# Arsham-001/tsu-emulator

Hardware: AMD Instinct MI355X
Metric: spin-updates/sec on L×L 2D Ising Gibbs sweep; achieved HBM GB/s vs peak (higher is better)
Workload: dtype int8

## Files before the change

tsu-emulator_amd/csrc/ising2d_tiled.hip:

```cpp
#include "ising2d.h"

#include <type_traits>
#include <vector>

typedef short v2s __attribute__((ext_vector_type(2)));
typedef unsigned short v2us __attribute__((ext_vector_type(2)));

struct TiledParams {
    const int8_t* src;
    int8_t* dst;
    long long pitch;
    int rows, nchunks;
    int cols;
    int q_shift;
    int tile_h;
    int flex_ty;
    int r_begin, r_end;
    long long row0, total_rows;
    int wrap_rows, ghost;
    int k;
    int tiles_x;
    int ty_first, ty_stride;
    uint32_t k0, k1, sweep0, tag_hi, tag_lo;
    uint32_t tblH0, tblH1, tblL0, tblL1;
    uint32_t t3H0, t3H1, t3L0, t3L1;
    int open;
    uint64_t thr[25];
};

static __device__ __forceinline__ uint32_t perm(uint32_t s0, uint32_t s1, uint32_t sel) {
    return __builtin_amdgcn_perm(s0, s1, sel);
}
static __device__ __forceinline__ uint32_t subsat16(uint32_t a, uint32_t b) {
    return __builtin_bit_cast(uint32_t, __builtin_elementwise_sub_sat(__builtin_bit_cast(v2s, a), __builtin_bit_cast(v2s, b)));
}
static __device__ __forceinline__ uint32_t minu16(uint32_t a, uint32_t b) {
    return __builtin_bit_cast(uint32_t, __builtin_elementwise_min(__builtin_bit_cast(v2us, a), __builtin_bit_cast(v2us, b)));
}

static __device__ __noinline__ u32x4 resolve_ties(u32x4 d, u32x4 w, uint32_t cnt_lo, uint32_t cnt_hi, const uint64_t* s_thr,
                                                  uint32_t cq, uint32_t Rg, uint32_t hs, uint32_t tag_lo, uint32_t k0,
                                                  uint32_t k1, uint32_t edge = 0) {
    const u32x4 l = tsu_philox(cq, Rg, hs, tag_lo, k0, k1);
#define TSU_FIX(DW, WW, LW, CNT, B0, M0)                                                                        \
    _Pragma("unroll") for (int hlf = 0; hlf < 2; ++hlf) {                                                       \
        const uint32_t sh = 16u * hlf;                                                                          \
        if (((DW >> sh) & 0xFFFFu) == 0) {                                                                      \
            const uint32_t c = (CNT >> (8 * (B0 + hlf))) & 0xFFu;                                               \
            const uint32_t m = M0 + hlf;                                                                        \
            const uint32_t deg = 4u - (edge & 1u) - ((m == 0 && (edge & 2u)) ? 1u : 0u) - ((m == (edge >> 4) && (edge & 4u)) ? 1u : 0u); \
            const uint64_t u = ((uint64_t)(((WW >> sh) & 0xFFFFu) ^ 0x8000u) << 16) | ((LW >> sh) & 0xFFFFu);   \
            const uint32_t f = (u < s_thr[deg * 5 + c]) ? 0x8000u : 0x0001u;       \
            DW = (DW & ~(0xFFFFu << sh)) | (f << sh);                                                           \
        }                                                                                                       \
    }
    TSU_FIX(d.x, w.x, l.x, cnt_lo, 0, 0)
    TSU_FIX(d.y, w.y, l.y, cnt_lo, 2, 2)
    TSU_FIX(d.z, w.z, l.z, cnt_hi, 0, 4)
    TSU_FIX(d.w, w.w, l.w, cnt_hi, 2, 6)
#undef TSU_FIX
    return d;
}

struct PhiloxKeys {
    uint32_t a[10], b[10];
};

static __device__ __forceinline__ PhiloxKeys make_keys(uint32_t k0, uint32_t k1) {
    PhiloxKeys K;
#pragma unroll
    for (int r = 0; r < 10; ++r) {
        uint32_t x = k0 + (uint32_t)r * TSU_PHILOX_W0, y = k1 + (uint32_t)r * TSU_PHILOX_W1;
        asm volatile("v_mov_b32 %0, %1" : "=v"(x) : "s"(x));
        asm volatile("v_mov_b32 %0, %1" : "=v"(y) : "s"(y));
        K.a[r] = x;
        K.b[r] = y;
    }
    return K;
}

static __device__ __forceinline__ u32x4 philox_vk(uint32_t c0, uint32_t c1, uint32_t c2, uint32_t c3, const PhiloxKeys& K) {
#pragma unroll
    for (int r = 0; r < 10; ++r) {
        uint64_t p0 = (uint64_t)TSU_PHILOX_M0 * c0;
        uint64_t p1 = (uint64_t)TSU_PHILOX_M1 * c2;
        uint32_t n0 = tsu_xor3((uint32_t)(p1 >> 32), c1, K.a[r]);
        uint32_t n2 = tsu_xor3((uint32_t)(p0 >> 32), c3, K.b[r]);
        c1 = (uint32_t)p1;
        c3 = (uint32_t)p0;
        c0 = n0;
        c2 = n2;
    }
    return u32x4{c0, c1, c2, c3};
}

struct Rows2Ctx {
    const void* Ps;
    void* Pd;
    const uint64_t* s_thr;
    int tr_lo, npairs;
    int rgf;
    int total_rows;
    int rg_tile0, wrap_tr;
    uint32_t hs, tag_hi, tag_lo, k0, k1;
    uint32_t tblH0, tblH1, tblL0, tblL1;
    uint32_t t3H0, t3H1, t3L0, t3L1;
    int last_row;
    bool lft, rgt;
    uint32_t r_par, r_slot;
    uint32_t rm_lo, rm_hi;
    uint64_t vm_e, vm_o;
    int sh_next, sh_prev;
};

static __device__ __forceinline__ u32x4 compare_octet(const u32x4& w, uint32_t cnt_lo, uint32_t cnt_hi, uint32_t tH0,
                                                      uint32_t tH1, uint32_t tL0, uint32_t tL1) {
    const uint32_t Hl = perm(tH1, tH0, cnt_lo), Ll = perm(tL1, tL0, cnt_lo);
    const uint32_t Hh = perm(tH1, tH0, cnt_hi), Lh = perm(tL1, tL0, cnt_hi);
    u32x4 d;
    d.x = subsat16(w.x, perm(Hl, Ll, 0x05010400u));
    d.y = subsat16(w.y, perm(Hl, Ll, 0x07030602u));
    d.z = subsat16(w.z, perm(Hh, Lh, 0x05010400u));
    d.w = subsat16(w.w, perm(Hh, Lh, 0x07030602u));
    return d;
}

static __device__ __forceinline__ u32x4 compare_octet_open(const u32x4& w, uint32_t cnt_lo, uint32_t cnt_hi, const Rows2Ctx& c,
                                                           bool row_edge, bool l0, bool r7) {
    uint32_t Hl = perm(c.tblH1, c.tblH0, cnt_lo), Ll = perm(c.tblL1, c.tblL0, cnt_lo);
    uint32_t Hh = perm(c.tblH1, c.tblH0, cnt_hi), Lh = perm(c.tblL1, c.tblL0, cnt_hi);
    if (row_edge | l0 | r7) {
        const uint32_t rl = r7 ? c.rm_lo : 0u, rh = r7 ? c.rm_hi : 0u;
        const uint32_t il = cnt_lo + ((row_edge && l0) ? 0x00000004u : 0u) + (row_edge ? (rl & 0x04040404u) : 0u);
        const uint32_t ih = cnt_hi + (row_edge ? (rh & 0x04040404u) : 0u);
        const uint32_t ml = row_edge ? 0xFFFFFFFFu : ((l0 ? 0x000000FFu : 0u) | rl), mh = row_edge ? 0xFFFFFFFFu : rh;
        Hl = (Hl & ~ml) | (perm(c.t3H1, c.t3H0, il) & ml);
        Ll = (Ll & ~ml) | (perm(c.t3L1, c.t3L0, il) & ml);
        Hh = (Hh & ~mh) | (perm(c.t3H1, c.t3H0, ih) & mh);
        Lh = (Lh & ~mh) | (perm(c.t3L1, c.t3L0, ih) & mh);
    }
    u32x4 d;
    d.x = subsat16(w.x, perm(Hl, Ll, 0x05010400u));
    d.y = subsat16(w.y, perm(Hl, Ll, 0x07030602u));
    d.z = subsat16(w.z, perm(Hh, Lh, 0x05010400u));
    d.w = subsat16(w.w, perm(Hh, Lh, 0x07030602u));
    return d;
}

static __device__ __forceinline__ bool has_zero_field(const u32x4& d) {
    const uint32_t mn = minu16(minu16(d.x, d.y), minu16(d.z, d.w));
    return ((mn & 0xFFFFu) == 0) | ((mn >> 16) == 0);
}

static __device__ __forceinline__ uint64_t pack_flags(const u32x4& d) {
    const uint32_t nlo = perm(d.y, d.x, 0x0B0A0908u) & 0x01010101u;
    const uint32_t nhi = perm(d.w, d.z, 0x0B0A0908u) & 0x01010101u;
    return (uint64_t)nlo | ((uint64_t)nhi << 32);
}

template <int NO>
static __device__ __forceinline__ void edge_rows(const Rows2Ctx& c, int to_wrap, int tr, int& rga, int& rgb) {
    constexpr int SPAN = 2 * ((NO - 1 + 63) / NO) + 1;
    const int s_off = to_wrap > 0 ? c.rg_tile0 : c.rg_tile0 - c.total_rows;
    rga = tr + s_off;
    rgb = rga + 1;
    if (__builtin_expect((uint32_t)(to_wrap - 1) < (uint32_t)SPAN, 0)) {
        rga = tr + c.rg_tile0;
        asm volatile("" : "+v"(rga));
        rgb = rga + 1;
        if (rga >= c.total_rows) rga -= c.total_rows;
        if (rgb >= c.total_rows) rgb -= c.total_rows;
    }
}

template <int NO, int P0, bool EDGE, bool OPEN, bool SEAM = false>
static __device__ __forceinline__ void sweep_pairs(const Rows2Ctx& c, const PhiloxKeys& K, int tr_first, int tr_end, int step_rows, int oct,
                                                   uint32_t cq) {
    const char* const ps0 = reinterpret_cast<const char*>(c.Ps);
    const int d_off = (int)(reinterpret_cast<const char*>(c.Pd) - ps0);
    const int off_end = tr_end * NO * 8;
    const int off_step = step_rows * NO * 8;
    int off = (tr_first * NO + oct) * 8;
    int rg = EDGE ? tr_first : c.rgf + (tr_first - c.tr_lo);
    int to_wrap = EDGE ? c.wrap_tr - __builtin_amdgcn_readfirstlane(rg) : 0;
#pragma unroll 1
    for (; off < off_end; off += off_step, rg += step_rows, to_wrap -= step_rows) {
        asm volatile("" : "+v"(off), "+v"(rg));
        const char* ps = ps0 + off;
        const uint64_t R0 = *reinterpret_cast<const uint64_t*>(ps - NO * 8), R1 = *reinterpret_cast<const uint64_t*>(ps);
        const uint64_t R2 = *reinterpret_cast<const uint64_t*>(ps + NO * 8), R3 = *reinterpret_cast<const uint64_t*>(ps + 2 * NO * 8);
        const uint32_t A0 = SEAM ? 0u : *reinterpret_cast<const uint32_t*>(ps + (P0 ? 8 : -4));
        const uint32_t A1 = SEAM ? 0u : *reinterpret_cast<const uint32_t*>(ps + NO * 8 + (P0 ? -4 : 8));
        const uint64_t Na = SEAM ? *reinterpret_cast<const uint64_t*>(ps + (P0 ? 8 : -8)) : 0ull;
        const uint64_t Nb = SEAM ? *reinterpret_cast<const uint64_t*>(ps + NO * 8 + (P0 ? -8 : 8)) : 0ull;
        __builtin_amdgcn_sched_barrier(0);
        int rga = rg, rgb = rg + 1;
        if (EDGE) edge_rows<NO>(c, to_wrap, rg, rga, rgb);
        const u32x4 w0 = philox_vk(cq, (uint32_t)rga, c.hs, c.tag_hi, K);
        const u32x4 w1 = philox_vk(cq, (uint32_t)rgb, c.hs, c.tag_hi, K);
        __builtin_amdgcn_sched_barrier(0);
        const uint32_t C0l = (uint32_t)R1, C0h = (uint32_t)(R1 >> 32), C1l = (uint32_t)R2, C1h = (uint32_t)(R2 >> 32);
        uint32_t S0l = P0 ? __builtin_amdgcn_alignbyte(C0h, C0l, 1) : __builtin_amdgcn_alignbyte(C0l, A0, 3);
        uint32_t S0h = P0 ? __builtin_amdgcn_alignbyte(A0, C0h, 1) : __builtin_amdgcn_alignbyte(C0h, C0l, 3);
        uint32_t S1l = P0 ? __builtin_amdgcn_alignbyte(C1l, A1, 3) : __builtin_amdgcn_alignbyte(C1h, C1l, 1);
        uint32_t S1h = P0 ? __builtin_amdgcn_alignbyte(C1h, C1l, 3) : __builtin_amdgcn_alignbyte(A1, C1h, 1);
        if (SEAM) {
            const uint64_t nxa = (Na & 0xFFull) << c.sh_next, pva = (Na >> c.sh_prev) & 0xFFull;
            const uint64_t nxb = (Nb & 0xFFull) << c.sh_next, pvb = (Nb >> c.sh_prev) & 0xFFull;
            const uint64_t Sa = P0 ? ((R1 >> 8) | nxa) : ((R1 << 8) | pva);
            const uint64_t Sb = P0 ? ((R2 << 8) | pvb) : ((R2 >> 8) | nxb);
            S0l = (uint32_t)Sa; S0h = (uint32_t)(Sa >> 32);
            S1l = (uint32_t)Sb; S1h = (uint32_t)(Sb >> 32);
        }
        const uint32_t ml = C0l + C1l, mh = C0h + C1h;
        const uint32_t cnt0l = (uint32_t)R0 + ml + S0l, cnt0h = (uint32_t)(R0 >> 32) + mh + S0h;
        const uint32_t cnt1l = (uint32_t)R3 + ml + S1l, cnt1h = (uint32_t)(R3 >> 32) + mh + S1h;
        u32x4 d0, d1;
        uint32_t edge_a = 0, edge_b = 0;
        if (OPEN) {
            const bool ea = rga == 0 || rga == c.last_row, eb = rgb == 0 || rgb == c.last_row;
            const bool la = !P0 && c.lft, ra = c.rgt && c.r_par == (uint32_t)P0, lb = P0 && c.lft, rb = c.rgt && c.r_par != (uint32_t)P0;
            d0 = compare_octet_open(w0, cnt0l, cnt0h, c, ea, la, ra);
            d1 = compare_octet_open(w1, cnt1l, cnt1h, c, eb, lb, rb);
            edge_a = (ea ? 1u : 0u) | (la ? 2u : 0u) | (ra ? 4u : 0u) | (c.r_slot << 4);
            edge_b = (eb ? 1u : 0u) | (lb ? 2u : 0u) | (rb ? 4u : 0u) | (c.r_slot << 4);
        } else {
            d0 = compare_octet(w0, cnt0l, cnt0h, c.tblH0, c.tblH1, c.tblL0, c.tblL1);
            d1 = compare_octet(w1, cnt1l, cnt1h, c.tblH0, c.tblH1, c.tblL0, c.tblL1);
        }
        const uint32_t mn = minu16(minu16(minu16(d0.x, d0.y), minu16(d0.z, d0.w)), minu16(minu16(d1.x, d1.y), minu16(d1.z, d1.w)));
        if (__builtin_expect(((mn & 0xFFFFu) == 0) | ((mn >> 16) == 0), 0)) {
            if (has_zero_field(d0)) d0 = resolve_ties(d0, w0, cnt0l, cnt0h, c.s_thr, cq, (uint32_t)rga, c.hs, c.tag_lo, c.k0, c.k1, edge_a);
            if (has_zero_field(d1)) d1 = resolve_ties(d1, w1, cnt1l, cnt1h, c.s_thr, cq, (uint32_t)rgb, c.hs, c.tag_lo, c.k0, c.k1, edge_b);
        }
        char* pd = const_cast<char*>(ps) + d_off;
        uint64_t n0 = pack_flags(d0), n1 = pack_flags(d1);
        if (OPEN) {
            n0 = (rga < 0 || rga > c.last_row) ? 0 : (n0 & (P0 ? c.vm_o : c.vm_e));
            n1 = (rgb < 0 || rgb > c.last_row) ? 0 : (n1 & (P0 ? c.vm_e : c.vm_o));
        }
        if (SEAM) {
            n0 &= c.vm_e;
            n1 &= c.vm_e;
        }
        *reinterpret_cast<uint64_t*>(pd) = n0;
        *reinterpret_cast<uint64_t*>(pd + NO * 8) = n1;
    }
}


static __device__ __forceinline__ uint32_t nib_shift_next(uint32_t X, uint32_t N) {
    const uint32_t hi = (N << 4) | __builtin_amdgcn_ubfe(X, 4u, 4u);
    return __builtin_amdgcn_alignbit(hi, X, 8);
}
static __device__ __forceinline__ uint32_t nib_shift_prev(uint32_t X, uint32_t M) {
    const uint32_t w = ((X << 4) & 0x10000000u) | (M >> 4);
    return __builtin_amdgcn_alignbit(X, w, 24);
}
static __device__ __forceinline__ uint32_t nib_shift_next_seam(uint32_t X, uint32_t N, int pos) {
    return nib_shift_next(X, 0u) | ((N & 0xFu) << pos);
}
static __device__ __forceinline__ uint32_t nib_shift_prev_seam(uint32_t X, uint32_t M, int pos) {
    const uint32_t w = ((X << 4) & 0x10000000u) | (((M >> pos) & 0xFu) << 24);
    return __builtin_amdgcn_alignbit(X, w, 24);
}
static __device__ __forceinline__ uint32_t nib_pack(const u32x4& d) {
    const uint64_t f = pack_flags(d);
    return (uint32_t)f | ((uint32_t)(f >> 32) << 4);
}

template <int NO, int P0, bool EDGE, bool OPEN = false, bool SEAM = false>
static __device__ __forceinline__ void sweep_pairs_nib(const Rows2Ctx& c, const PhiloxKeys& K, int tr_first, int tr_end, int step_rows, int oct,
                                                       uint32_t cq) {
    const char* const ps0 = reinterpret_cast<const char*>(c.Ps);
    const int d_off = (int)(reinterpret_cast<const char*>(c.Pd) - ps0);
    const int off_end = tr_end * NO * 4;
    const int off_step = step_rows * NO * 4;
    int off = (tr_first * NO + oct) * 4;
    int rg = EDGE ? tr_first : c.rgf + (tr_first - c.tr_lo);
    int to_wrap = EDGE ? c.wrap_tr - __builtin_amdgcn_readfirstlane(rg) : 0;
#pragma unroll 1
    for (; off < off_end; off += off_step, rg += step_rows, to_wrap -= step_rows) {
        asm volatile("" : "+v"(off), "+v"(rg));
        const char* ps = ps0 + off;
        const uint32_t R0 = *reinterpret_cast<const uint32_t*>(ps - NO * 4), R1 = *reinterpret_cast<const uint32_t*>(ps);
        const uint32_t R2 = *reinterpret_cast<const uint32_t*>(ps + NO * 4), R3 = *reinterpret_cast<const uint32_t*>(ps + 2 * NO * 4);
        const uint32_t A0 = *reinterpret_cast<const uint32_t*>(ps + (P0 ? 4 : -4));
        const uint32_t A1 = *reinterpret_cast<const uint32_t*>(ps + NO * 4 + (P0 ? -4 : 4));
        __builtin_amdgcn_sched_barrier(0);
        int rga = rg, rgb = rg + 1;
        if (EDGE) edge_rows<NO>(c, to_wrap, rg, rga, rgb);
        const u32x4 w0 = philox_vk(cq, (uint32_t)rga, c.hs, c.tag_hi, K);
        const u32x4 w1 = philox_vk(cq, (uint32_t)rgb, c.hs, c.tag_hi, K);
        __builtin_amdgcn_sched_barrier(0);
        const uint32_t Sa = SEAM ? (P0 ? nib_shift_next_seam(R1, A0, c.sh_next) : nib_shift_prev_seam(R1, A0, c.sh_prev))
                                 : (P0 ? nib_shift_next(R1, A0) : nib_shift_prev(R1, A0));
        const uint32_t Sb = SEAM ? (P0 ? nib_shift_prev_seam(R2, A1, c.sh_prev) : nib_shift_next_seam(R2, A1, c.sh_next))
                                 : (P0 ? nib_shift_prev(R2, A1) : nib_shift_next(R2, A1));
        const uint32_t mid = R1 + R2;
        const uint32_t cnt0 = R0 + mid + Sa, cnt1 = R3 + mid + Sb;
        const uint32_t cnt0l = cnt0 & 0x0F0F0F0Fu, cnt0h = (cnt0 >> 4) & 0x0F0F0F0Fu;
        const uint32_t cnt1l = cnt1 & 0x0F0F0F0Fu, cnt1h = (cnt1 >> 4) & 0x0F0F0F0Fu;
        u32x4 d0, d1;
        uint32_t edge_a = 0, edge_b = 0;
        if (OPEN) {
            const bool ea = rga == 0 || rga == c.last_row, eb = rgb == 0 || rgb == c.last_row;
            const bool la = !P0 && c.lft, ra = c.rgt && c.r_par == (uint32_t)P0, lb = P0 && c.lft, rb = c.rgt && c.r_par != (uint32_t)P0;
            d0 = compare_octet_open(w0, cnt0l, cnt0h, c, ea, la, ra);
            d1 = compare_octet_open(w1, cnt1l, cnt1h, c, eb, lb, rb);
            edge_a = (ea ? 1u : 0u) | (la ? 2u : 0u) | (ra ? 4u : 0u) | (c.r_slot << 4);
            edge_b = (eb ? 1u : 0u) | (lb ? 2u : 0u) | (rb ? 4u : 0u) | (c.r_slot << 4);
        } else {
            d0 = compare_octet(w0, cnt0l, cnt0h, c.tblH0, c.tblH1, c.tblL0, c.tblL1);
            d1 = compare_octet(w1, cnt1l, cnt1h, c.tblH0, c.tblH1, c.tblL0, c.tblL1);
        }
        const uint32_t mn = minu16(minu16(minu16(d0.x, d0.y), minu16(d0.z, d0.w)), minu16(minu16(d1.x, d1.y), minu16(d1.z, d1.w)));
        if (__builtin_expect(((mn & 0xFFFFu) == 0) | ((mn >> 16) == 0), 0)) {
            if (has_zero_field(d0)) d0 = resolve_ties(d0, w0, cnt0l, cnt0h, c.s_thr, cq, (uint32_t)rga, c.hs, c.tag_lo, c.k0, c.k1, edge_a);
            if (has_zero_field(d1)) d1 = resolve_ties(d1, w1, cnt1l, cnt1h, c.s_thr, cq, (uint32_t)rgb, c.hs, c.tag_lo, c.k0, c.k1, edge_b);
        }
        char* pd = const_cast<char*>(ps) + d_off;
        uint32_t n0 = nib_pack(d0), n1 = nib_pack(d1);
        if (OPEN) {
            const uint64_t ma = P0 ? c.vm_o : c.vm_e, mb = P0 ? c.vm_e : c.vm_o;
            n0 = (rga < 0 || rga > c.last_row) ? 0u : (n0 & ((uint32_t)ma | ((uint32_t)(ma >> 32) << 4)));
            n1 = (rgb < 0 || rgb > c.last_row) ? 0u : (n1 & ((uint32_t)mb | ((uint32_t)(mb >> 32) << 4)));
        }
        if (SEAM) {
            const uint32_t m = (uint32_t)c.vm_e | ((uint32_t)(c.vm_e >> 32) << 4);
            n0 &= m;
            n1 &= m;
        }
        *reinterpret_cast<uint32_t*>(pd) = n0;
        *reinterpret_cast<uint32_t*>(pd + NO * 4) = n1;
    }
}

static __device__ __forceinline__ void xst(uint64_t* p, uint64_t v) { __hip_atomic_store(p, v, __ATOMIC_RELAXED, __HIP_MEMORY_SCOPE_AGENT); }
static __device__ __forceinline__ uint64_t xld(const uint64_t* p) { return __hip_atomic_load(p, __ATOMIC_RELAXED, __HIP_MEMORY_SCOPE_AGENT); }

struct ResidentParams {
    uint64_t* xbuf;
    uint32_t gen0;
    int* err;
    int n_gen, k_last, tiles_y;
    int wrap_y;
    int wrap_x;
    long long* dbg;
};

template <int HT, int WO, int THREADS, bool OPEN = false, bool RESIDENT = false, bool NIB = false>
static __device__ __forceinline__ void tile_body(const TiledParams& p, const int8_t* __restrict__ src, int8_t* __restrict__ dst,
                                                 const int k, const uint32_t sweep0, const int tx, const int ty, uint64_t* lds,
                                                 const PhiloxKeys& K, const ResidentParams* R = nullptr) {
    constexpr int NO = WO + 2;
    constexpr int RLMAX = THREADS / NO;
    int H = p.tile_h, row_off = ty * p.tile_h;
    if (p.flex_ty > 0) {
        const long long half = (p.r_end - p.r_begin + 1) / 2;
        row_off = 2 * (int)(ty * half / p.flex_ty);
        H = 2 * (int)((ty + 1) * half / p.flex_ty) - row_off;
    }
    const int TR = H + 4 * k;
    constexpr int RL = RLMAX;
    using E = typename std::conditional<NIB, uint32_t, uint64_t>::type;
    E* plane0 = reinterpret_cast<E*>(lds + 1);
    E* plane1 = plane0 + TR * NO;
    uint64_t* s_thr = reinterpret_cast<uint64_t*>((reinterpret_cast<uintptr_t>(plane1 + TR * NO + NO + 1) + 7u) & ~(uintptr_t)7u);
    const int tid = threadIdx.x;
    if (tid < 25) s_thr[tid] = p.thr[tid];

    const int q0 = tx * WO + p.q_shift, r0 = p.r_begin + row_off, Rb = r0 - 2 * k;

    const int al = tid / NO, oct = tid - al * NO;
    int cqi = q0 - 1 + oct;
    const bool col_out = OPEN && (cqi < 0 || cqi >= p.nchunks);
    if (!OPEN) {
        if (cqi < 0) cqi += p.nchunks;
        if (cqi >= p.nchunks) cqi -= p.nchunks;
        if (cqi >= p.nchunks) cqi -= p.nchunks;
    }
    const uint32_t cq = (uint32_t)cqi;
    int nv = p.cols - 16 * cqi;
    if (col_out) nv = 0;
    if (nv > 16) nv = 16;
    auto first_sites = [](int n) { return n >= 8 ? 0x0101010101010101ull : (((1ull << (8 * n)) - 1) & 0x0101010101010101ull); };
    const uint64_t vm_e = first_sites((nv + 1) >> 1), vm_o = first_sites(nv >> 1);

    if (al < RLMAX) {
        const int8_t* col = src + 16 * (long long)(OPEN ? (cqi < 0 ? 0 : (cqi >= p.nchunks ? p.nchunks - 1 : cqi)) : cqi);
        constexpr int LB = 4;
        for (int tr0 = al; tr0 < TR; tr0 += LB * RLMAX) {
            uint4 v[LB];
#pragma unroll
            for (int b = 0; b < LB; ++b) {
                const int tr = tr0 + b * RLMAX;
                const int rl = Rb + (tr < TR ? tr : TR - 1);
                int srow;
                if (p.wrap_rows) srow = rl < 0 ? rl + p.rows : (rl >= p.rows ? rl - p.rows : rl);
                else srow = rl < -p.ghost ? -p.ghost : (rl >= p.rows + p.ghost ? p.rows + p.ghost - 1 : rl);
                v[b] = *reinterpret_cast<const uint4*>(col + (long long)srow * p.pitch);
            }
#pragma unroll
            for (int b = 0; b < LB; ++b) {
                const int tr = tr0 + b * RLMAX;
                if (tr < TR) {
                    const uint32_t e0 = perm(v[b].y, v[b].x, 0x06040200u), e1 = perm(v[b].w, v[b].z, 0x06040200u);
                    const uint32_t o0 = perm(v[b].y, v[b].x, 0x07050301u), o1 = perm(v[b].w, v[b].z, 0x07050301u);
                    uint64_t ev = (uint64_t)(~(e0 >> 1) & 0x01010101u) | ((uint64_t)(~(e1 >> 1) & 0x01010101u) << 32);
                    uint64_t od = (uint64_t)(~(o0 >> 1) & 0x01010101u) | ((uint64_t)(~(o1 >> 1) & 0x01010101u) << 32);
                    if (OPEN) {
                        const long long grow = p.row0 + Rb + tr;
                        if (grow < 0 || grow >= p.total_rows) ev = od = 0;
                    }
                    if (OPEN || nv < 16) {
                        ev &= vm_e;
                        od &= vm_o;
                    }
                    const int idx = tr * NO + oct;
                    const int gpar = (int)((p.row0 + Rb + tr) & 1);
                    if (NIB) {
                        (gpar ? plane1 : plane0)[idx] = (E)((uint32_t)ev | ((uint32_t)(ev >> 32) << 4));
                        (gpar ? plane0 : plane1)[idx] = (E)((uint32_t)od | ((uint32_t)(od >> 32) << 4));
                    } else {
                        (gpar ? plane1 : plane0)[idx] = (E)ev;
                        (gpar ? plane0 : plane1)[idx] = (E)od;
                    }
                }
            }
        }
    }

    long long rg0 = p.row0 + Rb;
    if (!OPEN) {
        rg0 %= p.total_rows;
        if (rg0 < 0) rg0 += p.total_rows;
    }
    const bool edge = !OPEN && (rg0 + TR > p.total_rows);

    Rows2Ctx c;
    c.s_thr = s_thr;
    c.total_rows = (int)p.total_rows;
    c.rg_tile0 = (int)rg0;
    c.wrap_tr = (int)(p.total_rows - rg0);
    c.tag_hi = p.tag_hi; c.tag_lo = p.tag_lo; c.k0 = p.k0; c.k1 = p.k1;
    c.tblH0 = p.tblH0; c.tblH1 = p.tblH1; c.tblL0 = p.tblL0; c.tblL1 = p.tblL1;
    c.t3H0 = p.t3H0; c.t3H1 = p.t3H1; c.t3L0 = p.t3L0; c.t3L1 = p.t3L1;
    c.last_row = (int)p.total_rows - 1;
    c.lft = OPEN && cqi == 0;
    c.rgt = OPEN && cqi == p.nchunks - 1;
    c.r_par = (uint32_t)(p.cols - 1) & 1u;
    c.r_slot = ((uint32_t)(p.cols - 1) & 15u) >> 1;
    c.rm_lo = c.r_slot < 4 ? 0xFFu << (8 * c.r_slot) : 0u;
    c.rm_hi = c.r_slot < 4 ? 0u : 0xFFu << (8 * (c.r_slot - 4));
    c.vm_e = vm_e;
    c.vm_o = vm_o;
    const int v_last = (p.cols >> 1) & 7;
    const bool ragged = !OPEN && v_last != 0;
    const int seam_site = v_last - 1;
    const int seam_pos = NIB ? 8 * (seam_site & 3) + 4 * (seam_site >> 2) : 8 * seam_site, last_pos = NIB ? 28 : 56;
    c.sh_next = (ragged && cqi == p.nchunks - 1) ? seam_pos : last_pos;
    c.sh_prev = (ragged && cqi == 0) ? seam_pos : last_pos;
    int w0 = (q0 - 1) % p.nchunks;
    if (w0 < 0) w0 += p.nchunks;
    const bool seam = ragged && (w0 == 0 || w0 + NO - 1 >= p.nchunks - 1);
    asm volatile("v_mov_b32 %0, %1" : "=v"(c.tblH0) : "s"(p.tblH0));
    asm volatile("v_mov_b32 %0, %1" : "=v"(c.tblH1) : "s"(p.tblH1));
    asm volatile("v_mov_b32 %0, %1" : "=v"(c.tblL0) : "s"(p.tblL0));
    asm volatile("v_mov_b32 %0, %1" : "=v"(c.tblL1) : "s"(p.tblL1));

    const int n_gen = RESIDENT ? R->n_gen : 1;
    long long tl0 = 0, tl[4] = {0, 0, 0, 0};
    const bool timing = RESIDENT && R->dbg && tid == 0;
    if (timing) tl0 = wall_clock64();
#define RES_MARK(q)                         \
    if (timing) {                           \
        const long long now_ = wall_clock64(); \
        tl[q] += now_ - tl0;                \
        tl0 = now_;                         \
    }
    volatile int& s_fail = *reinterpret_cast<volatile int*>(lds);
    if (RESIDENT && tid == 0) s_fail = 0;

    const int n_tb = 2 * k * WO, n_lr = H;
    const int xstride = 2 * n_tb + 2 * p.tile_h;
    const int wi = (p.nchunks + p.q_shift - q0) < WO ? (p.nchunks + p.q_shift - q0) : WO;
    constexpr uint64_t TAG_MASK = NIB ? 0xFFFFFFFF00000000ull : 0xFEFEull, FLAG_MASK = NIB ? 0x11111111ull : 0x0101010101010101ull;
    auto strip_tag = [&](int gen) -> uint64_t {
        const uint32_t G = R->gen0 + (uint32_t)gen;
        return NIB ? ((uint64_t)G << 32) : (((uint64_t)(G & 0x7Fu) << 1) | ((uint64_t)((G >> 7) & 0x7Fu) << 9));
    };
    auto publish = [&](int gen) {
        RES_MARK(0);
        const int ntiles = p.tiles_x * R->tiles_y, me = ty * p.tiles_x + tx;
        uint64_t* mine = R->xbuf + ((size_t)(gen & 1) * ntiles + me) * xstride;
        const uint64_t tag = strip_tag(gen);
        for (int i = tid; i < n_tb; i += THREADS) {
            const int r = i / WO, o = i - r * WO;
            xst(mine + i, (uint64_t)plane1[(2 * k + r) * NO + 1 + o] | tag);
            xst(mine + n_tb + i, (uint64_t)plane1[(H + r) * NO + 1 + o] | tag);
        }
        for (int i = tid; i < n_lr; i += THREADS) {
            xst(mine + 2 * n_tb + i, (uint64_t)plane1[(2 * k + i) * NO + 1] | tag);
            xst(mine + 2 * n_tb + n_lr + i, (uint64_t)plane1[(2 * k + i) * NO + wi] | tag);
        }
        RES_MARK(1);
    };
    auto fetch = [&](int gen) {
        RES_MARK(0);
        const int tiles_x = p.tiles_x, tiles_y = R->tiles_y, ntiles = tiles_x * tiles_y;
        const uint64_t tag = strip_tag(gen);
        const int txl = tx == 0 ? tiles_x - 1 : tx - 1, txr = tx == tiles_x - 1 ? 0 : tx + 1;
        const int w_l = txl == tiles_x - 1 ? p.nchunks + p.q_shift - (txl * WO + p.q_shift) : WO;
        const int tyu = ty == 0 ? tiles_y - 1 : ty - 1, tyd = ty == tiles_y - 1 ? 0 : ty + 1;
        const bool has_u = R->wrap_y || ty > 0, has_d = R->wrap_y || ty < tiles_y - 1;
        const bool has_l = R->wrap_x || tx > 0, has_r = R->wrap_x || tx < tiles_x - 1;
        const uint64_t* xg = R->xbuf + (size_t)(gen & 1) * ntiles * xstride;
        const uint64_t* X_u = xg + (size_t)(tyu * tiles_x + tx) * xstride;
        const uint64_t* X_d = xg + (size_t)(tyd * tiles_x + tx) * xstride;
        const uint64_t* X_l = xg + (size_t)(ty * tiles_x + txl) * xstride;
        const uint64_t* X_r = xg + (size_t)(ty * tiles_x + txr) * xstride;
        const uint64_t* X_ul = xg + (size_t)(tyu * tiles_x + txl) * xstride;
        const uint64_t* X_ur = xg + (size_t)(tyu * tiles_x + txr) * xstride;
        const uint64_t* X_dl = xg + (size_t)(tyd * tiles_x + txl) * xstride;
        const uint64_t* X_dr = xg + (size_t)(tyd * tiles_x + txr) * xstride;
        constexpr int FI = (2 * 8 * NO + THREADS - 1) / THREADS;
        constexpr int TH_MAX = 160 * 1024 / (int)sizeof(E) / (2 * NO) - 32;
        constexpr int SI = (TH_MAX + THREADS - 1) / THREADS;
        const uint64_t* au[FI];
        const uint64_t* ad[FI];
        uint64_t vu[FI], vd[FI], vl[SI], vr[SI];
        bool nu[FI], nd[FI], nl[SI], nr[SI];
#pragma unroll
        for (int it = 0; it < FI; ++it) {
            const int i = tid + it * THREADS, ic = i < 2 * k * NO ? i : 0;
            const int r = ic / NO, o = ic - r * NO;
            const int e = r * WO;
            const int oc = o <= wi + 1 ? o : 1;
            au[it] = oc == 0 ? X_ul + n_tb + e + w_l - 1 : (oc == wi + 1 ? X_ur + n_tb + e : X_u + n_tb + e + oc - 1);
            ad[it] = oc == 0 ? X_dl + e + w_l - 1 : (oc == wi + 1 ? X_dr + e : X_d + e + oc - 1);
            const bool col_ok = o == 0 ? has_l : (o == wi + 1 ? has_r : o <= wi);
            nu[it] = i < 2 * k * NO && has_u && col_ok;
            nd[it] = i < 2 * k * NO && has_d && col_ok;
            vu[it] = xld(au[it]);
            vd[it] = xld(ad[it]);
        }
#pragma unroll
        for (int it = 0; it < SI; ++it) {
            const int i = tid + it * THREADS, ic = i < n_lr ? i : 0;
            nl[it] = i < n_lr && has_l;
            nr[it] = i < n_lr && has_r;
            vl[it] = xld(X_l + 2 * n_tb + n_lr + ic);
            vr[it] = xld(X_r + 2 * n_tb + ic);
        }
        for (int spins = 0;; ++spins) {
            bool fresh = true;
#pragma unroll
            for (int it = 0; it < FI; ++it) {
                if (nu[it] && (vu[it] & TAG_MASK) != tag) { vu[it] = xld(au[it]); fresh = false; }
                if (nd[it] && (vd[it] & TAG_MASK) != tag) { vd[it] = xld(ad[it]); fresh = false; }
            }
#pragma unroll
            for (int it = 0; it < SI; ++it) {
                const int i = tid + it * THREADS, ic = i < n_lr ? i : 0;
                if (nl[it] && (vl[it] & TAG_MASK) != tag) { vl[it] = xld(X_l + 2 * n_tb + n_lr + ic); fresh = false; }
                if (nr[it] && (vr[it] & TAG_MASK) != tag) { vr[it] = xld(X_r + 2 * n_tb + ic); fresh = false; }
            }
            if (fresh) break;
            if (spins > (1 << 22) || ((spins & 0xFFF) == 0xFFF && __hip_atomic_load(R->err, __ATOMIC_RELAXED, __HIP_MEMORY_SCOPE_SYSTEM))) {
                __hip_atomic_store(R->err, 1, __ATOMIC_RELAXED, __HIP_MEMORY_SCOPE_SYSTEM);
                s_fail = 1;
                break;
            }
        }
        RES_MARK(2);
#pragma unroll
        for (int it = 0; it < FI; ++it) {
            const int i = tid + it * THREADS;
            if (i < 2 * k * NO) {
                const int r = i / NO, o = i - r * NO;
                if (nu[it]) plane1[r * NO + o] = (E)(vu[it] & FLAG_MASK);
                if (nd[it]) plane1[(2 * k + H + r) * NO + o] = (E)(vd[it] & FLAG_MASK);
            }
        }
#pragma unroll
        for (int it = 0; it < SI; ++it) {
            const int i = tid + it * THREADS;
            if (i < n_lr) {
                if (nl[it]) plane1[(2 * k + i) * NO] = (E)(vl[it] & FLAG_MASK);
                if (nr[it]) plane1[(2 * k + i) * NO + wi + 1] = (E)(vr[it] & FLAG_MASK);
            }
        }
        RES_MARK(3);
    };

    auto run = [&](int par0, int tr_first, int tr_end, int step, int oc, uint32_t cqq) {
        if (NIB && OPEN) {
            if (par0) sweep_pairs_nib<NO, 1, false, true>(c, K, tr_first, tr_end, step, oc, cqq);
            else sweep_pairs_nib<NO, 0, false, true>(c, K, tr_first, tr_end, step, oc, cqq);
        } else if (NIB && seam) {
            if (par0) sweep_pairs_nib<NO, 1, true, false, true>(c, K, tr_first, tr_end, step, oc, cqq);
            else sweep_pairs_nib<NO, 0, true, false, true>(c, K, tr_first, tr_end, step, oc, cqq);
        } else if (NIB) {
            if (edge) {
                if (par0) sweep_pairs_nib<NO, 1, true>(c, K, tr_first, tr_end, step, oc, cqq);
                else sweep_pairs_nib<NO, 0, true>(c, K, tr_first, tr_end, step, oc, cqq);
            } else {
                if (par0) sweep_pairs_nib<NO, 1, false>(c, K, tr_first, tr_end, step, oc, cqq);
                else sweep_pairs_nib<NO, 0, false>(c, K, tr_first, tr_end, step, oc, cqq);
            }
        } else if (OPEN) {
            if (par0) sweep_pairs<NO, 1, false, true>(c, K, tr_first, tr_end, step, oc, cqq);
            else sweep_pairs<NO, 0, false, true>(c, K, tr_first, tr_end, step, oc, cqq);
        } else if (seam) {
            if (par0) sweep_pairs<NO, 1, true, false, true>(c, K, tr_first, tr_end, step, oc, cqq);
            else sweep_pairs<NO, 0, true, false, true>(c, K, tr_first, tr_end, step, oc, cqq);
        } else if (edge) {
            if (par0) sweep_pairs<NO, 1, true, false>(c, K, tr_first, tr_end, step, oc, cqq);
            else sweep_pairs<NO, 0, true, false>(c, K, tr_first, tr_end, step, oc, cqq);
        } else {
            if (par0) sweep_pairs<NO, 1, false, false>(c, K, tr_first, tr_end, step, oc, cqq);
            else sweep_pairs<NO, 0, false, false>(c, K, tr_first, tr_end, step, oc, cqq);
        }
    };
    int par0 = 0;
    auto set_half_sweep = [&](uint32_t sweep_g, int hsi) {
        const int kappa = hsi & 1;
        c.hs = 2u * (sweep_g + (uint32_t)(hsi >> 1)) + (uint32_t)kappa;
        c.Pd = kappa ? plane1 : plane0;
        c.Ps = kappa ? plane0 : plane1;
        c.tr_lo = 1 + hsi;
        c.npairs = (TR - 2 - 2 * hsi) / 2;
        int rgf = (int)rg0 + c.tr_lo;
        if (!OPEN && rgf >= c.total_rows) rgf -= c.total_rows;
        c.rgf = rgf;
        par0 = (int)((p.row0 + Rb + c.tr_lo + kappa) & 1);
    };
    for (int gen = 0; gen < n_gen; ++gen) {
    const int kg = (RESIDENT && gen == n_gen - 1) ? R->k_last : k;
    const uint32_t sweep_g = sweep0 + (uint32_t)(gen * k);
    for (int hsi = 0; hsi < 2 * kg; ++hsi) {
        __syncthreads();
        set_half_sweep(sweep_g, hsi);
        if (al < RL) run(par0, c.tr_lo + 2 * al, c.tr_lo + 2 * c.npairs, 2 * RL, oct, cq);
    }
    __syncthreads();
    if (RESIDENT && gen + 1 < n_gen) {
        publish(gen);
        fetch(gen);
        __syncthreads();
        if (s_fail) return;
    }
    RES_MARK(0);
    }
    if (timing)
        for (int q = 0; q < 4; ++q) R->dbg[4 * blockIdx.x + q] = tl[q];
#undef RES_MARK
    if (al < RLMAX && oct >= 1 && oct <= WO && q0 + oct - 1 < p.nchunks + p.q_shift) {
        int8_t* col = dst + 16 * (long long)cqi;
        int gpar = (int)((p.row0 + r0 + al) & 1);
#pragma unroll 2
        for (int hr = al; hr < H; hr += RLMAX) {
            const int rl = r0 + hr;
            if (rl < p.r_end) {
                const int li = (2 * k + hr) * NO + oct;
                uint64_t ev = (gpar ? plane1 : plane0)[li], od = (gpar ? plane0 : plane1)[li];
                if (NIB) {
                    ev = (ev & 0x01010101ull) | (((ev >> 4) & 0x01010101ull) << 32);
                    od = (od & 0x01010101ull) | (((od >> 4) & 0x01010101ull) << 32);
                }
                const uint32_t e0 = perm(0u, 0x000001FFu, (uint32_t)ev), e1 = perm(0u, 0x000001FFu, (uint32_t)(ev >> 32));
                const uint32_t o0 = perm(0u, 0x000001FFu, (uint32_t)od), o1 = perm(0u, 0x000001FFu, (uint32_t)(od >> 32));
                uint4 v = make_uint4(perm(o0, e0, 0x05010400u), perm(o0, e0, 0x07030602u), perm(o1, e1, 0x05010400u),
                                     perm(o1, e1, 0x07030602u));
                if (nv < 16) {
                    auto bytes = [](int n) { return n >= 4 ? 0xFFFFFFFFu : (n <= 0 ? 0u : (1u << (8 * n)) - 1u); };
                    v.x &= bytes(nv);
                    v.y &= bytes(nv - 4);
                    v.z &= bytes(nv - 8);
                    v.w &= bytes(nv - 12);
                }
                *reinterpret_cast<uint4*>(col + (long long)rl * p.pitch) = v;
            }
            if (RLMAX & 1) gpar ^= 1;
        }
    }
}

template <int H, int WO, int THREADS, int MINW = 1, bool OPEN = false, bool NIB = false>
__global__ __launch_bounds__(THREADS, MINW) void k1_tiled2(TiledParams p) {
    extern __shared__ uint64_t lds[];
    const PhiloxKeys K = make_keys(p.k0, p.k1);
    tile_body<H, WO, THREADS, OPEN, false, NIB>(p, p.src, p.dst, p.k, p.sweep0, blockIdx.x % p.tiles_x,
                                    p.ty_first + (blockIdx.x / p.tiles_x) * p.ty_stride, lds, K);
}

struct ResidentLaunch {
    TiledParams t;
    ResidentParams r;
};

template <int H, int WO, int THREADS, int MINW = 1, bool OPEN = false, bool NIB = false>
__global__ __launch_bounds__(THREADS, MINW) void k1_resident(ResidentLaunch P) {
    extern __shared__ uint64_t lds[];
    const PhiloxKeys K = make_keys(P.t.k0, P.t.k1);
    tile_body<H, WO, THREADS, OPEN, true, NIB>(P.t, P.t.src, P.t.dst, P.t.k, P.t.sweep0, blockIdx.x % P.t.tiles_x, blockIdx.x / P.t.tiles_x,
                                          lds, K, &P.r);
}

namespace {
constexpr int KMAX = 8;

struct TileVariant {
    int H, WO, threads;
    void (*kernel)(TiledParams);
    void (*resident)(ResidentLaunch);
    void (*open)(TiledParams);
    void (*resident_open)(ResidentLaunch);
    int nib;
    int per_cu;
};

size_t tile_lds_bytes(const TileVariant& tv, int TR) {
    const size_t es = tv.nib ? 4 : 8, NO = (size_t)tv.WO + 2;
    return 8 + (((size_t)2 * TR * NO + NO + 1) * es + 7) / 8 * 8 + 8 + 25 * sizeof(uint64_t);
}
enum { V_64x512_T512 = 0, V_128x512_T512, V_128x512_T1024, V_256x512_T1024, V_128x256_T1024, V_64x512_T1024, V_64x256_T1024, V_32x256_T1024,
       V_N512x512_T1024, V_N256x512_T512 };
const TileVariant kVariants[] = {
    {64, 32, 512, k1_tiled2<64, 32, 512>, k1_resident<64, 32, 512>, k1_tiled2<64, 32, 512, 1, true>, nullptr, 0, 2},
    {128, 32, 512, k1_tiled2<128, 32, 512>, k1_resident<128, 32, 512>, k1_tiled2<128, 32, 512, 1, true>, nullptr, 0, 2},
    {128, 32, 1024, k1_tiled2<128, 32, 1024>, k1_resident<128, 32, 1024>, k1_tiled2<128, 32, 1024, 1, true>, k1_resident<128, 32, 1024, 1, true>, 0, 1},
    {256, 32, 1024, k1_tiled2<256, 32, 1024, 4>, k1_resident<256, 32, 1024, 4>, k1_tiled2<256, 32, 1024, 4, true>, k1_resident<256, 32, 1024, 4, true>, 0, 1},
    {128, 16, 1024, k1_tiled2<128, 16, 1024>, k1_resident<128, 16, 1024>, k1_tiled2<128, 16, 1024, 1, true>, k1_resident<128, 16, 1024, 1, true>, 0, 1},
    {64, 32, 1024, k1_tiled2<64, 32, 1024>, k1_resident<64, 32, 1024>, k1_tiled2<64, 32, 1024, 1, true>, k1_resident<64, 32, 1024, 1, true>, 0, 1},
    {64, 16, 1024, k1_tiled2<64, 16, 1024>, k1_resident<64, 16, 1024>, k1_tiled2<64, 16, 1024, 1, true>, k1_resident<64, 16, 1024, 1, true>, 0, 1},
    {32, 16, 1024, k1_tiled2<32, 16, 1024>, k1_resident<32, 16, 1024>, k1_tiled2<32, 16, 1024, 1, true>, k1_resident<32, 16, 1024, 1, true>, 0, 1},
    {512, 32, 1024, k1_tiled2<512, 32, 1024, 4, false, true>, k1_resident<512, 32, 1024, 4, false, true>, k1_tiled2<512, 32, 1024, 4, true, true>,
     k1_resident<512, 32, 1024, 4, true, true>, 1, 1},
    {256, 32, 512, k1_tiled2<256, 32, 512, 4, false, true>, nullptr, k1_tiled2<256, 32, 512, 4, true, true>, nullptr, 1, 2},
};
constexpr int kNumVariants = sizeof(kVariants) / sizeof(kVariants[0]);

int ragged_shift(const tsu_ising2d* L, int WO) {
    if (!L->periodic || L->cols % 16 == 0) return 0;
    const int nch = (L->cols + 15) / 16, tiles_x = (nch + WO - 1) / WO;
    for (int shift = 1; shift < WO && shift < nch - 1; ++shift) {
        bool ok = true;
        for (int t = 0; t < tiles_x && ok; ++t) {
            const int s = t * WO + shift;
            if (s % nch == 0) ok = false;
            if (t < tiles_x - 1 && (s + WO) % nch == nch - 1) ok = false;
        }
        if (ok) return shift;
    }
    return -1;
}

size_t lds_share(const TileVariant& tv) { return (size_t)(160 / tv.per_cu) * 1024; }

int chip_cus(const tsu_ising2d* L) { return L->ctx->cus > 0 ? L->ctx->cus : 256; }

int lattice_env(const char* name, int dflt) {
    const char* e = getenv(name);
    return e ? atoi(e) : dflt;
}

double gen_time_us(const TileVariant& c, int h, double between) {
    const int pairs = (h + 4 * 8 - 2) / 2, waves = (pairs * (c.WO + 2) + 63) / 64;
    return 16.0 * (0.25 + (c.nib ? 1.06 : 1.0) * 0.225 * ((waves + 3) / 4)) + between;
}

template <typename P>
void pack_thresholds(P& p, const uint64_t table[25]) {
    for (int c = 0; c < 25; ++c) p.thr[c] = table[c];
    auto top16 = [](uint64_t thr) {
        uint32_t thi = (uint32_t)(thr >> 16);
        if (thi > 65535u) thi = 65535u;
        return thi ^ 0x8000u;
    };
    uint32_t t16[5], t3[8] = {0, 0, 0, 0, 0, 0, 0, 0};
    for (int c = 0; c < 5; ++c) t16[c] = top16(table[4 * 5 + c]);
    for (int c = 0; c < 4; ++c) t3[c] = top16(table[3 * 5 + c]);
    for (int c = 0; c < 3; ++c) t3[4 + c] = top16(table[2 * 5 + c]);
    p.t3L0 = (t3[0] & 0xFF) | ((t3[1] & 0xFF) << 8) | ((t3[2] & 0xFF) << 16) | ((t3[3] & 0xFF) << 24);
    p.t3L1 = (t3[4] & 0xFF) | ((t3[5] & 0xFF) << 8) | ((t3[6] & 0xFF) << 16);
    p.t3H0 = (t3[0] >> 8) | ((t3[1] >> 8) << 8) | ((t3[2] >> 8) << 16) | ((t3[3] >> 8) << 24);
    p.t3H1 = (t3[4] >> 8) | ((t3[5] >> 8) << 8) | ((t3[6] >> 8) << 16);
    p.tblL0 = (t16[0] & 0xFF) | ((t16[1] & 0xFF) << 8) | ((t16[2] & 0xFF) << 16) | ((t16[3] & 0xFF) << 24);
    p.tblL1 = (t16[4] & 0xFF);
    p.tblH0 = (t16[0] >> 8) | ((t16[1] >> 8) << 8) | ((t16[2] >> 8) << 16) | ((t16[3] >> 8) << 24);
    p.tblH1 = (t16[4] >> 8);
}

int flex_cut(const tsu_ising2d* L, int v, int* v_out, int* hmax_out, double* t_out) {
    if (L->ghost != 0 || L->total_rows != L->rows) return 0;
    if (L->periodic && ((L->cols & 1) || (L->rows & 1))) return 0;
    const int FLEX_HMIN = 16;
    static const int max_tiles = lattice_env("TSU_K1_FLEX_MAX_TILES", 0);
    int cus = chip_cus(L);
    if (max_tiles > 0 && max_tiles < cus) cus = max_tiles;
    const int nch = (L->cols + 15) / 16;
    static const int cand[] = {V_256x512_T1024, V_128x256_T1024, V_N512x512_T1024};
    double best = 1e300;
    int best_ty = 0;
    for (int ci = 0; ci < (int)(sizeof(cand) / sizeof(cand[0])); ++ci) {
        if (v >= 0 && cand[ci] != v) continue;
        const TileVariant& c = kVariants[cand[ci]];
        if (!(L->periodic ? c.resident : c.resident_open) || 2 * nch < c.WO || ragged_shift(L, c.WO) < 0) continue;
        const int tiles_x = (nch + c.WO - 1) / c.WO, half = (L->rows + 1) / 2;
        int tiles_y = cus / tiles_x;
        if (tiles_y > half / (FLEX_HMIN / 2)) tiles_y = half / (FLEX_HMIN / 2);
        if (tiles_y < 1) continue;
        const int hmax = 2 * ((half + tiles_y - 1) / tiles_y), hmin = 2 * (half / tiles_y);
        if (hmin < FLEX_HMIN || L->total_rows < hmax + 4 * KMAX || tile_lds_bytes(c, hmax + 4 * KMAX) > 160 * 1024) continue;
        const double t_gen = gen_time_us(c, hmax, 4.3);
        if (t_gen < best) {
            best = t_gen;
            best_ty = tiles_y;
            *v_out = cand[ci];
            *hmax_out = hmax;
        }
    }
    *t_out = best;
    return best_ty;
}

struct CallPlan {
    int v;
    int flex_ty, flex_h;
    int kmax;
    bool resident;
    int tile_h, tiles_y;
    int res_ext;
};

CallPlan plan_call(const tsu_ising2d* L, int n_sweeps, int part) {
    CallPlan c{};
    static const int env = lattice_env("TSU_TILE_VARIANT", -1);
    const bool forced = env >= 0 && env < kNumVariants;
    const int cus = chip_cus(L), nch = (L->cols + 15) / 16;
    const bool whole_lattice = L->ghost == 0 && L->total_rows == L->rows;
    int v;
    if (forced) {
        v = env;
    } else {
        const long long tx = (nch + 31) / 32;
        const long long n128 = ((L->rows + 127) / 128) * tx, n256 = ((L->rows + 255) / 256) * tx;
        if (n128 <= cus) v = V_128x512_T1024;
        else if (n128 <= 2 * cus && n256 <= cus && 10 * n256 >= 7 * cus) v = V_256x512_T1024;
        else v = V_128x512_T512;
        if (L->rows < 256) v = V_64x512_T512;
        if (whole_lattice && n128 > 2 * cus) {
            const long long n512 = (long long)(L->rows / 512) * (nch / 32);
            if (L->rows % 512 == 0 && nch % 32 == 0 && n512 <= cus && 2 * n512 > cus) v = V_N512x512_T1024;
            else if (L->rows >= 512) v = V_N256x512_T512;
        }
        static const int cand[] = {V_256x512_T1024, V_128x512_T1024, V_128x256_T1024, V_64x512_T1024, V_64x256_T1024, V_32x256_T1024};
        double best = 1e30;
        for (int ci = 0; whole_lattice && ci < (int)(sizeof(cand) / sizeof(cand[0])); ++ci) {
            const TileVariant& t = kVariants[cand[ci]];
            if (!(L->periodic ? t.kernel : t.open)) continue;
            if (2 * nch < t.WO || L->total_rows < t.H + 4 * KMAX || ragged_shift(L, t.WO) < 0) continue;
            const long long nt = (long long)((L->rows + t.H - 1) / t.H) * ((nch + t.WO - 1) / t.WO);
            if (nt > cus) continue;
            const bool resident = (L->periodic ? t.resident : t.resident_open) && L->rows % t.H == 0 && nch % t.WO == 0;
            const double t_gen = gen_time_us(t, t.H, resident ? 4.3 : 12.0);
            if (t_gen < best) {
                best = t_gen;
                v = cand[ci];
            }
        }
    }
    {
        const TileVariant& t = kVariants[v];
        const long long nt = (long long)((L->rows + t.H - 1) / t.H) * ((nch + t.WO - 1) / t.WO);
        const bool divides = L->rows % t.H == 0 && nch % t.WO == 0;
        const bool standard_resident = (L->periodic ? t.resident : t.resident_open) && divides && nt <= (long long)t.per_cu * cus;
        int fv = -1, fh = 0;
        double t_flex = 0;
        const int fty = forced ? (divides ? 0 : flex_cut(L, v, &fv, &fh, &t_flex)) : flex_cut(L, -1, &fv, &fh, &t_flex);
        bool take = fty > 0 && !standard_resident;
        const bool compact = L->ctx->in_batch && 2 * nt <= cus;
        if (compact) take = false;
        if (fty > 0 && standard_resident && !forced && t.per_cu == 1 && !compact) take = t_flex < 0.97 * gen_time_us(t, t.H, 4.3);
        if (take) {
            v = fv;
            c.flex_ty = fty;
            c.flex_h = fh;
        }
    }
    auto fits = [&](int vv) {
        return 2 * nch >= kVariants[vv].WO && L->total_rows >= kVariants[vv].H + 4 * KMAX && (L->periodic || kVariants[vv].open) &&
               ragged_shift(L, kVariants[vv].WO) >= 0;
    };
    if (!fits(v)) {
        static const int fallback[] = {V_64x512_T512, V_64x256_T1024, V_32x256_T1024};
        v = -1;
        c.flex_ty = c.flex_h = 0;
        for (int f : fallback)
            if (fits(f)) {
                v = f;
                break;
            }
    }
    c.v = v;
    if (v < 0) return c;

    const TileVariant& tv = kVariants[v];
    c.kmax = L->sweeps_per_launch > 0 ? L->sweeps_per_launch : ((tv.nib || tv.threads >= 1024 || (long long)L->rows * L->cols <= 4096ll * 4096ll) ? 8 : 5);
    if (c.kmax > KMAX) c.kmax = KMAX;
    c.tile_h = tv.H;
    c.tiles_y = (L->rows + tv.H - 1) / tv.H;
    static const int use_resident = lattice_env("TSU_K1_RESIDENT", 1);
    c.resident = use_resident && (L->periodic ? tv.resident : tv.resident_open) && part == TSU_PART_ALL && n_sweeps > c.kmax;
    const bool whole = L->wrap_rows || (!L->periodic && whole_lattice);
    if (!c.resident) return c;
    if (whole && c.flex_ty > 0) {
        c.tile_h = c.flex_h;
        c.tiles_y = c.flex_ty;
    } else if (whole) {
        c.resident = nch % tv.WO == 0 && L->rows % tv.H == 0;
    } else {
        const int need = L->rows + 4 * (n_sweeps - c.kmax);
        int th = (need + c.tiles_y - 1) / c.tiles_y;
        th += th & 1;
        if (th < tv.H) th = tv.H;
        const int extra = th * c.tiles_y - L->rows;
        c.tile_h = th;
        c.res_ext = extra / 2;
        c.resident = nch % tv.WO == 0 && extra % 2 == 0 && c.res_ext <= L->ghost && tile_lds_bytes(tv, th + 4 * c.kmax) <= lds_share(tv);
    }
    return c;
}

int launch_tiles(const tsu_ising2d* L, const TileVariant& tv, int k, int left, int part, bool slab, TiledParams& p) {
    p.tile_h = tv.H;
    p.r_begin = 0;
    p.r_end = L->rows;
    if (part != TSU_PART_ALL) return (L->rows + tv.H - 1) / tv.H;
    if (!slab) {
        const long long slots = (long long)tv.per_cu * chip_cus(L);
        double best = 1e300;
        for (int th = 32; th <= 1024; th += 2) {
            if (th + 4 * KMAX > L->total_rows || tile_lds_bytes(tv, th + 4 * k) > lds_share(tv)) continue;
            const long long nt = (long long)((L->rows + th - 1) / th) * p.tiles_x, rounds = (nt + slots - 1) / slots;
            const double cost = (double)rounds * (th + 2 * k + 12);
            if (cost < best * (1.0 - 1e-9) || (cost <= best * (1.0 + 1e-9) && th > p.tile_h)) {
                best = cost;
                p.tile_h = th;
            }
        }
        return (L->rows + p.tile_h - 1) / p.tile_h;
    }
    const int ext = 2 * (left - k);
    p.r_begin = -ext;
    p.r_end = L->rows + ext;
    const int base_ty = (L->rows + tv.H - 1) / tv.H;
    int th = (p.r_end - p.r_begin + base_ty - 1) / base_ty;
    th += th & 1;
    if (th >= tv.H && tile_lds_bytes(tv, th + 4 * k) <= lds_share(tv)) p.tile_h = th;
    return (p.r_end - p.r_begin + p.tile_h - 1) / p.tile_h;
}

void print_resident_timeline(const long long* d_dbg, int ntiles, int tiles_x, int tiles_y, int n_gen, int verbose) {
    std::vector<long long> h((size_t)4 * ntiles);
    (void)hipMemcpy(h.data(), d_dbg, h.size() * sizeof(long long), hipMemcpyDeviceToHost);
    static const char* const what[4] = {"sweeps", "publish", "wait", "fetch"};
    fprintf(stderr, "[tsu]   us per generation over %d tiles (mean / min / max):", ntiles);
    for (int q = 0; q < 4; ++q) {
        double sum = 0, lo = 1e30, hi = 0;
        for (int t = 0; t < ntiles; ++t) {
            const double v = h[(size_t)4 * t + q] / 100.0 / n_gen;
            sum += v;
            lo = v < lo ? v : lo;
            hi = v > hi ? v : hi;
        }
        fprintf(stderr, " %s %.1f / %.1f / %.1f%s", what[q], sum / ntiles, lo, hi, q < 3 ? "," : "\n");
    }
    if (verbose < 3) return;
    for (int x = 0; x < 8; ++x) {
        double sw = 0, wt = 0;
        int cnt = 0;
        for (int t = x; t < ntiles; t += 8, ++cnt) {
            sw += h[(size_t)4 * t] / 100.0 / n_gen;
            wt += h[(size_t)4 * t + 2] / 100.0 / n_gen;
        }
        if (cnt) fprintf(stderr, "[tsu]   xcd %d: sweeps %.2f wait %.2f\n", x, sw / cnt, wt / cnt);
    }
    if (verbose < 4) return;
    for (int y = 0; y < tiles_y; ++y) {
        fprintf(stderr, "[tsu]   row %3d:", y);
        for (int x = 0; x < tiles_x; ++x)
            fprintf(stderr, " %.1f/%.1f", h[(size_t)4 * (y * tiles_x + x)] / 100.0 / n_gen, h[(size_t)4 * (y * tiles_x + x) + 2] / 100.0 / n_gen);
        fprintf(stderr, "\n");
    }
}

int run_resident(tsu_ising2d* L, const CallPlan& c, TiledParams p, int n_sweeps, uint32_t sweep0, int fit_per_cu) {
    tsu_ctx* ctx = L->ctx;
    const TileVariant& tv = kVariants[c.v];
    void (*const res_kern)(ResidentLaunch) = L->periodic ? tv.resident : tv.resident_open;
    const int kmax = c.kmax, ntiles = p.tiles_x * c.tiles_y;
    const bool whole = L->wrap_rows || (!L->periodic && L->ghost == 0 && L->total_rows == L->rows);
    const size_t lds_bytes = tile_lds_bytes(tv, c.tile_h + 4 * kmax);
    const size_t xstride = (size_t)2 * (2 * kmax * tv.WO) + (size_t)2 * c.tile_h;
    const size_t xneed = (size_t)2 * ntiles * xstride;
    if (L->xbuf_cap < xneed * sizeof(uint64_t)) L->xsig = 0;
    TSU_HIP_TRY(ctx, ising2d_grow(L->d_xbuf, L->xbuf_cap, xneed * sizeof(uint64_t)));
    const uint64_t xsig = ((uint64_t)(c.v + 1) << 48) ^ ((uint64_t)ntiles << 28) ^ ((uint64_t)kmax << 20) ^ ((uint64_t)c.tile_h << 4) ^
                          ((uint64_t)c.flex_ty << 36) ^ (uint64_t)p.open;
    if (!L->h_err) {
        TSU_HIP_TRY(ctx, hipHostMalloc(&L->h_err, sizeof(int), hipHostMallocMapped));
        *L->h_err = 0;
    }
    int* d_err = nullptr;
    TSU_HIP_TRY(ctx, hipHostGetDevicePointer((void**)&d_err, L->h_err, 0));
    const int verbose = lattice_env("TSU_K1_VERBOSE", 0);
    const int chunk_max = whole ? 1024 * kmax : n_sweeps;
    for (int done = 0; done < n_sweeps;) {
        const int chunk = n_sweeps - done < chunk_max ? n_sweeps - done : chunk_max;
        ResidentLaunch P;
        p.k = kmax;
        p.sweep0 = sweep0 + (uint32_t)done;
        p.ty_first = 0;
        p.ty_stride = 1;
        p.src = L->alloc[L->cur] + (size_t)L->ghost * L->pitch;
        p.dst = L->alloc[L->cur ^ 1] + (size_t)L->ghost * L->pitch;
        p.tile_h = c.tile_h;
        p.flex_ty = c.flex_ty;
        p.r_begin = -c.res_ext;
        p.r_end = L->rows + c.res_ext;
        P.t = p;
        P.r.wrap_y = L->wrap_rows ? 1 : 0;
        P.r.wrap_x = L->periodic ? 1 : 0;
        P.r.xbuf = L->d_xbuf;
        const bool renumber = L->xsig != xsig || L->xgen + (uint32_t)((chunk + kmax - 1) / kmax) + 2u >= 16383u;
        if (renumber) {
            L->xsig = xsig;
            L->xgen = 0;
        }
        P.r.gen0 = L->xgen + 1u;
        L->xgen += (uint32_t)((chunk + kmax - 1) / kmax);
        P.r.err = d_err;
        P.r.n_gen = (chunk + kmax - 1) / kmax;
        P.r.k_last = chunk - (P.r.n_gen - 1) * kmax;
        P.r.tiles_y = c.tiles_y;
        P.r.dbg = nullptr;
        long long* d_dbg = nullptr;
        if (verbose >= 2) {
            TSU_HIP_TRY(ctx, hipMalloc(&d_dbg, (size_t)4 * ntiles * sizeof(long long)));
            P.r.dbg = d_dbg;
        }
        if (verbose)
            fprintf(stderr, "[tsu] k1_resident variant %d: %d tiles (%d per CU fit), %d generations of %d sweeps, %zu KB of strips\n",
                    c.v, ntiles, fit_per_cu, P.r.n_gen, kmax, xneed * 8 / 1024);
        {
            const int rcx = tsu_grid_exclusive_begin(ctx);
            if (rcx != TSU_OK) return rcx;
        }
        if (renumber) TSU_HIP_TRY(ctx, hipMemsetAsync(L->d_xbuf, 0, L->xbuf_cap, ctx->stream));
        TSU_HIP_TRY(ctx, tsu_launch_grid_sync(ctx, (const void*)res_kern, dim3((unsigned)ntiles), dim3((unsigned)tv.threads), &P, lds_bytes, ctx->stream,
                                              !whole));
        L->launches += 1;
        L->cur ^= 1;
        {
            const int rcx = tsu_grid_exclusive_end(ctx);
            if (rcx != TSU_OK) return rcx;
        }
        if (d_dbg) {
            print_resident_timeline(d_dbg, ntiles, p.tiles_x, c.tiles_y, P.r.n_gen, verbose);
            (void)hipFree(d_dbg);
        }
        done += chunk;
    }
    return TSU_OK;
}

int run_generations(tsu_ising2d* L, const CallPlan& c, TiledParams p, int n_sweeps, uint32_t sweep0, int part) {
    tsu_ctx* ctx = L->ctx;
    const TileVariant& tv = kVariants[c.v];
    void (*const kern)(TiledParams) = L->periodic ? tv.kernel : tv.open;
    const bool slab = !(L->wrap_rows || (!L->periodic && L->ghost == 0 && L->total_rows == L->rows));
    for (int done = 0; done < n_sweeps;) {
        const int k = n_sweeps - done < c.kmax ? n_sweeps - done : c.kmax;
        p.k = k;
        p.sweep0 = sweep0 + (uint32_t)done;
        p.src = L->alloc[L->cur] + (size_t)L->ghost * L->pitch;
        p.dst = L->alloc[L->cur ^ 1] + (size_t)L->ghost * L->pitch;
        const int tiles_y = launch_tiles(L, tv, k, n_sweeps - done, part, slab, p);
        const size_t lds_bytes = tile_lds_bytes(tv, p.tile_h + 4 * k);
        int n_ty = tiles_y;
        p.ty_first = 0;
        p.ty_stride = 1;
        if (part == TSU_PART_INTERIOR) {
            p.ty_first = 1;
            n_ty = tiles_y - 2;
        } else if (part == TSU_PART_BOUNDARY && tiles_y >= 2) {
            p.ty_stride = tiles_y - 1;
            n_ty = 2;
        }
        if (n_ty > 0) {
            hipLaunchKernelGGL(kern, dim3((unsigned)(p.tiles_x * n_ty)), dim3((unsigned)tv.threads), lds_bytes, ctx->stream, p);
            L->launches += 1;
        }
        if (part != TSU_PART_INTERIOR) L->cur ^= 1;
        done += k;
    }
    TSU_HIP_TRY(ctx, hipGetLastError());
    return TSU_OK;
}
}

int tsu_ising2d_tiled_supported(const tsu_ising2d* L) {
    if (plan_call(L, 0, TSU_PART_ALL).v < 0) return 0;
    const bool open_whole = !L->periodic && L->ghost == 0 && L->total_rows == L->rows;
    if (!L->wrap_rows && !open_whole && L->ghost < 2) return 0;
    return 1;
}

int tsu_ising2d_tiled_tiles(const tsu_ising2d* L) {
    if (!tsu_ising2d_tiled_supported(L)) return 0;
    const CallPlan c = plan_call(L, 0, TSU_PART_ALL);
    const TileVariant& tv = kVariants[c.v];
    const int tiles_x = (((L->cols + 15) / 16) + tv.WO - 1) / tv.WO;
    return (c.flex_ty > 0 ? c.flex_ty : (L->rows + tv.H - 1) / tv.H) * tiles_x;
}

int tsu_ising2d_tiled_part_supported(const tsu_ising2d* L) {
    return tsu_ising2d_tiled_supported(L) && !L->wrap_rows && (L->rows % kVariants[plan_call(L, 0, TSU_PART_ALL).v].H) == 0;
}

int tsu_ising2d_tiled_sweep(tsu_ising2d* L, int n_sweeps, uint64_t seed, uint32_t sweep0, uint32_t replica, int part) {
    tsu_ctx* ctx = L->ctx;
    const CallPlan c = plan_call(L, n_sweeps, part);
    const TileVariant& tv = kVariants[c.v];
    if (!L->alloc[1]) {
        size_t bytes = (size_t)(L->rows + 2 * L->ghost) * L->pitch;
        TSU_HIP_TRY(ctx, hipMalloc(&L->alloc[1], bytes));
        TSU_HIP_TRY(ctx, hipMemsetAsync(L->alloc[1], 0, bytes, ctx->stream));
    }
    if (!L->wrap_rows && !(!L->periodic && L->ghost == 0 && L->total_rows == L->rows)) {
        TSU_REQUIRE(ctx, 2 * n_sweeps <= L->ghost, "ising2d_sweep (tiled, slab): %d sweeps per ghost refresh exceed ghost/2 = %d",
                    n_sweeps, L->ghost / 2);
        TSU_REQUIRE(ctx, part == TSU_PART_ALL || n_sweeps <= c.kmax, "ising2d_sweep_part: split sweeps take at most %d sweeps", c.kmax);
    }
    TiledParams p;
    p.pitch = (long long)L->pitch;
    p.rows = L->rows;
    p.nchunks = (L->cols + 15) / 16;
    p.cols = L->cols;
    p.row0 = L->row0;
    p.total_rows = L->total_rows;
    p.wrap_rows = L->wrap_rows;
    p.ghost = L->ghost;
    p.tiles_x = (p.nchunks + tv.WO - 1) / tv.WO;
    p.q_shift = ragged_shift(L, tv.WO);
    p.r_begin = 0;
    p.r_end = L->rows;
    p.tile_h = tv.H;
    p.flex_ty = 0;
    ising2d_set_keys(p, seed, replica);
    pack_thresholds(p, L->table);
    p.open = L->periodic ? 0 : 1;
    TSU_HIP_TRY(ctx, tsu_func_allow_lds(ctx, (const void*)(L->periodic ? tv.kernel : tv.open), 160 * 1024));
    if (c.resident) {
        void (*const res_kern)(ResidentLaunch) = L->periodic ? tv.resident : tv.resident_open;
        TSU_HIP_TRY(ctx, tsu_func_allow_lds(ctx, (const void*)res_kern, 160 * 1024));
        int fit_per_cu = 0;
        TSU_HIP_TRY(ctx, tsu_func_blocks_per_cu(ctx, (const void*)res_kern, tv.threads, tile_lds_bytes(tv, (c.flex_ty > 0 ? c.tile_h : tv.H) + 4 * KMAX),
                                                &fit_per_cu));
        if ((long long)p.tiles_x * c.tiles_y <= (long long)fit_per_cu * ctx->cus) return run_resident(L, c, p, n_sweeps, sweep0, fit_per_cu);
    }
    return run_generations(L, c, p, n_sweeps, sweep0, part);
}

struct PlanesItem {
    int8_t* buf;
    long long pitch;
    int rows, cols, periodic;
    uint32_t k0, k1, tag_hi, tag_lo, sweep0;
    uint32_t tblH0, tblH1, tblL0, tblL1, t3H0, t3H1, t3L0, t3L1;
    uint64_t thr[25];
};

template <bool OPEN>
__global__ __launch_bounds__(1024) void k1_planes(const PlanesItem* __restrict__ items, PlanesItem one, int n_sweeps) {
    __shared__ uint64_t s_planes[2 * 1024];
    __shared__ uint64_t s_thr[25];
    const PlanesItem& it = items ? items[blockIdx.x] : one;
    const int tid = threadIdx.x;
    const int rows = it.rows, cols = it.cols, nch = (cols + 15) >> 4, tasks = rows * nch;
    if (tid < 25) s_thr[tid] = it.thr[tid];
    const PhiloxKeys K = make_keys(it.k0, it.k1);
    const bool active = tid < tasks;
    const int r = active ? tid / nch : 0, q = active ? tid - r * nch : 0;
    const int idx = r * nch + q;
    uint64_t* const plane0 = s_planes;
    uint64_t* const plane1 = s_planes + tasks;
    int nv = cols - 16 * q;
    if (nv > 16) nv = 16;
    auto first_sites = [](int n) { return n >= 8 ? 0x0101010101010101ull : (((1ull << (8 * n)) - 1) & 0x0101010101010101ull); };
    const uint64_t vm_e = first_sites((nv + 1) >> 1), vm_o = first_sites(nv >> 1);
    int8_t* const chunk = it.buf + (long long)r * it.pitch + 16 * q;
    if (active) {
        const uint4 v = *reinterpret_cast<const uint4*>(chunk);
        const uint32_t e0 = perm(v.y, v.x, 0x06040200u), e1 = perm(v.w, v.z, 0x06040200u);
        const uint32_t o0 = perm(v.y, v.x, 0x07050301u), o1 = perm(v.w, v.z, 0x07050301u);
        uint64_t ev = (uint64_t)(~(e0 >> 1) & 0x01010101u) | ((uint64_t)(~(e1 >> 1) & 0x01010101u) << 32);
        uint64_t od = (uint64_t)(~(o0 >> 1) & 0x01010101u) | ((uint64_t)(~(o1 >> 1) & 0x01010101u) << 32);
        ev &= vm_e;
        od &= vm_o;
        ((r & 1) ? plane1 : plane0)[idx] = ev;
        ((r & 1) ? plane0 : plane1)[idx] = od;
    }
    const int up = r > 0 ? idx - nch : (OPEN ? -1 : idx + (rows - 1) * nch);
    const int dn = r < rows - 1 ? idx + nch : (OPEN ? -1 : idx - (rows - 1) * nch);
    const int lf = q > 0 ? idx - 1 : (OPEN ? -1 : idx + nch - 1);
    const int rt = q < nch - 1 ? idx + 1 : (OPEN ? -1 : idx - (nch - 1));
    const int v_last = ((cols >> 1) & 7) ? ((cols >> 1) & 7) : 8;
    const int shl = q == nch - 1 ? 8 * (v_last - 1) : 56, shr = q == 0 ? 8 * (v_last - 1) : 56;
    Rows2Ctx c;
    c.s_thr = s_thr;
    c.t3H0 = it.t3H0; c.t3H1 = it.t3H1; c.t3L0 = it.t3L0; c.t3L1 = it.t3L1;
    asm volatile("v_mov_b32 %0, %1" : "=v"(c.tblH0) : "s"(it.tblH0));
    asm volatile("v_mov_b32 %0, %1" : "=v"(c.tblH1) : "s"(it.tblH1));
    asm volatile("v_mov_b32 %0, %1" : "=v"(c.tblL0) : "s"(it.tblL0));
    asm volatile("v_mov_b32 %0, %1" : "=v"(c.tblL1) : "s"(it.tblL1));
    c.r_par = (uint32_t)(cols - 1) & 1u;
    c.r_slot = ((uint32_t)(cols - 1) & 15u) >> 1;
    c.rm_lo = c.r_slot < 4 ? 0xFFu << (8 * c.r_slot) : 0u;
    c.rm_hi = c.r_slot < 4 ? 0u : 0xFFu << (8 * (c.r_slot - 4));
    const bool row_edge = OPEN && (r == 0 || r == rows - 1);
    const uint32_t tag_hi = it.tag_hi, tag_lo = it.tag_lo, k0 = it.k0, k1 = it.k1, sweep0 = it.sweep0;
    for (int hsi = 0; hsi < 2 * n_sweeps; ++hsi) {
        __syncthreads();
        const int kappa = hsi & 1;
        const uint32_t hs = 2u * (sweep0 + (uint32_t)(hsi >> 1)) + (uint32_t)kappa;
        if (active) {
            const uint64_t* Ps = kappa ? plane0 : plane1;
            uint64_t* Pd = kappa ? plane1 : plane0;
            const int par = (r + kappa) & 1;
            const uint64_t U = (OPEN && up < 0) ? 0ull : Ps[up], D = (OPEN && dn < 0) ? 0ull : Ps[dn], C = Ps[idx];
            const int side = par ? rt : lf;
            const uint64_t A = (OPEN && side < 0) ? 0ull : Ps[side];
            const uint64_t S = par ? ((C >> 8) | ((A & 0xFFull) << shl)) : ((C << 8) | ((A >> shr) & 0xFFull));
            const uint64_t cnt = U + D + C + S;
            const uint32_t cnt_lo = (uint32_t)cnt, cnt_hi = (uint32_t)(cnt >> 32);
            const u32x4 w = philox_vk((uint32_t)q, (uint32_t)r, hs, tag_hi, K);
            u32x4 d;
            uint32_t edge = 0;
            if (OPEN) {
                const bool l0 = !par && q == 0, r7 = q == nch - 1 && c.r_par == (uint32_t)par;
                d = compare_octet_open(w, cnt_lo, cnt_hi, c, row_edge, l0, r7);
                edge = (row_edge ? 1u : 0u) | (l0 ? 2u : 0u) | (r7 ? 4u : 0u) | (c.r_slot << 4);
            } else {
                d = compare_octet(w, cnt_lo, cnt_hi, c.tblH0, c.tblH1, c.tblL0, c.tblL1);
            }
            if (__builtin_expect(has_zero_field(d), 0)) d = resolve_ties(d, w, cnt_lo, cnt_hi, s_thr, (uint32_t)q, (uint32_t)r, hs, tag_lo, k0, k1, edge);
            uint64_t n = pack_flags(d);
            n &= par ? vm_o : vm_e;
            Pd[idx] = n;
        }
    }
    __syncthreads();
    if (active) {
        const uint64_t ev = ((r & 1) ? plane1 : plane0)[idx], od = ((r & 1) ? plane0 : plane1)[idx];
        const uint32_t e0 = perm(0u, 0x000001FFu, (uint32_t)ev), e1 = perm(0u, 0x000001FFu, (uint32_t)(ev >> 32));
        const uint32_t o0 = perm(0u, 0x000001FFu, (uint32_t)od), o1 = perm(0u, 0x000001FFu, (uint32_t)(od >> 32));
        uint4 v = make_uint4(perm(o0, e0, 0x05010400u), perm(o0, e0, 0x07030602u), perm(o1, e1, 0x05010400u), perm(o1, e1, 0x07030602u));
        if (nv < 16) {
            auto bytes = [](int n) { return n >= 4 ? 0xFFFFFFFFu : (n <= 0 ? 0u : (1u << (8 * n)) - 1u); };
            v.x &= bytes(nv);
            v.y &= bytes(nv - 4);
            v.z &= bytes(nv - 8);
            v.w &= bytes(nv - 12);
        }
        *reinterpret_cast<uint4*>(chunk) = v;
    }
}

int tsu_ising2d_planes_supported(const tsu_ising2d* L) {
    if (L->ghost != 0 || L->total_rows != L->rows || L->row0 != 0) return 0;
    if ((long long)L->rows * ((L->cols + 15) / 16) > 1024) return 0;
    return L->rows >= 2 && L->cols >= 2;
}

int tsu_ising2d_planes_sweep(tsu_ising2d* const* lats, int n, int n_sweeps, const uint64_t* seeds, const uint32_t* sweep0s,
                             const uint32_t* replicas) {
    tsu_ctx* ctx = lats[0]->ctx;
    std::vector<PlanesItem> items((size_t)n);
    for (int i = 0; i < n; ++i) {
        const tsu_ising2d* L = lats[i];
        PlanesItem& it = items[(size_t)i];
        it.buf = L->alloc[L->cur] + (size_t)L->ghost * L->pitch;
        it.pitch = (long long)L->pitch;
        it.rows = L->rows;
        it.cols = L->cols;
        it.periodic = L->periodic;
        ising2d_set_keys(it, seeds[i], replicas[i]);
        it.sweep0 = sweep0s[i];
        pack_thresholds(it, L->table);
    }
    const tsu_ising2d* L0c = lats[0];
    const int tasks = L0c->rows * ((L0c->cols + 15) / 16);
    const unsigned threads = (unsigned)((tasks + 63) / 64 * 64);
    void (*const kern)(const PlanesItem*, PlanesItem, int) = L0c->periodic ? k1_planes<false> : k1_planes<true>;
    if (n == 1) {
        hipLaunchKernelGGL(kern, dim3(1), dim3(threads), 0, ctx->stream, (const PlanesItem*)nullptr, items[0], n_sweeps);
    } else {
        tsu_ising2d* L0 = lats[0];
        const size_t bytes = items.size() * sizeof(PlanesItem);
        TSU_HIP_TRY(ctx, ising2d_grow(L0->d_batch, L0->batch_cap, bytes));
        TSU_HIP_TRY(ctx, hipMemcpyAsync(L0->d_batch, items.data(), bytes, hipMemcpyHostToDevice, ctx->stream));
        TSU_HIP_TRY(ctx, hipStreamSynchronize(ctx->stream));
        hipLaunchKernelGGL(kern, dim3((unsigned)n), dim3(threads), 0, ctx->stream, (const PlanesItem*)L0->d_batch, items[0], n_sweeps);
    }
    TSU_HIP_TRY(ctx, hipGetLastError());
    for (int i = 0; i < n; ++i) lats[i]->launches += 1;
    return TSU_OK;
}
```

Before: 3017 billion.

## Interleave spin planes in LDS and template sweep loop on half-sweep parity

Replaces the two separate LDS planes with one interleaved layout where rows of both parities alternate, so each thread reaches neighbours through a single 32-bit LDS address plus compile-time offsets. The per-half-sweep state (source/dest pointers, hs, row bounds) moves out of the context struct and into template parameters (KAPPA) and a per-generation sweep driver. The loop walks a precomputed trip count with a tail predicate instead of comparing pointer offsets. The aim is to cut address arithmetic, 64-bit pointer handling and runtime dispatch inside the hot loop, at the cost of more template instantiations and possible register or code-size growth.

```diff
diff --git a/tsu-emulator_amd/csrc/ising2d_tiled.hip b/tsu-emulator_amd/csrc/ising2d_tiled.hip
--- a/tsu-emulator_amd/csrc/ising2d_tiled.hip
+++ b/tsu-emulator_amd/csrc/ising2d_tiled.hip
@@ -95,14 +95,10 @@
 }
 
 struct Rows2Ctx {
-    const void* Ps;
-    void* Pd;
     const uint64_t* s_thr;
-    int tr_lo, npairs;
-    int rgf;
     int total_rows;
     int rg_tile0, wrap_tr;
-    uint32_t hs, tag_hi, tag_lo, k0, k1;
+    uint32_t tag_hi, tag_lo, k0, k1;
     uint32_t tblH0, tblH1, tblL0, tblL1;
     uint32_t t3H0, t3H1, t3L0, t3L1;
     int last_row;
@@ -110,6 +106,7 @@
     uint32_t r_par, r_slot;
     uint32_t rm_lo, rm_hi;
     uint64_t vm_e, vm_o;
+    uint32_t nvm_e, nvm_o;
     int sh_next, sh_prev;
 };
 
@@ -173,78 +170,96 @@
     }
 }
 
-template <int NO, int P0, bool EDGE, bool OPEN, bool SEAM = false>
-static __device__ __forceinline__ void sweep_pairs(const Rows2Ctx& c, const PhiloxKeys& K, int tr_first, int tr_end, int step_rows, int oct,
+#define TSU_LDS __attribute__((address_space(3)))
+static __device__ __forceinline__ uint32_t lds_addr(const void* p) { return (uint32_t)(uintptr_t)(const TSU_LDS char*)p; }
+template <typename T>
+static __device__ __forceinline__ T lds_ld(uint32_t a) { return *(const TSU_LDS T*)(uintptr_t)a; }
+template <typename T>
+static __device__ __forceinline__ void lds_st(uint32_t a, T v) { *(TSU_LDS T*)(uintptr_t)a = v; }
+
+template <typename E, int NO>
+struct TilePlanes {
+    E* base;
+    __device__ __forceinline__ E& at(int pl, int r, int o) const { return base[(2 * r + pl) * NO + o]; }
+};
+
+template <int NO, int KAPPA, int P0, bool EDGE, bool OPEN, bool SEAM>
+static __device__ __forceinline__ void pair_step(const Rows2Ctx& c, const PhiloxKeys& K, uint32_t hs, uint32_t a, int rg, int to_wrap,
+                                                 uint32_t cq) {
+    constexpr int RS = 2 * NO * 8;
+    constexpr int DO = (KAPPA ? NO : -NO) * 8;
+    const uint64_t R0 = lds_ld<uint64_t>(a), R1 = lds_ld<uint64_t>(a + RS);
+    const uint64_t R2 = lds_ld<uint64_t>(a + 2 * RS), R3 = lds_ld<uint64_t>(a + 3 * RS);
+    const uint32_t A0 = SEAM ? 0u : (P0 ? lds_ld<volatile uint32_t>(a + RS + 8) : lds_ld<uint32_t>(a + RS - 4));
+    const uint32_t A1 = SEAM ? 0u : (P0 ? lds_ld<uint32_t>(a + 2 * RS - 4) : lds_ld<volatile uint32_t>(a + 2 * RS + 8));
+    const uint64_t Na = SEAM ? lds_ld<uint64_t>(a + RS + (P0 ? 8 : -8)) : 0ull;
+    const uint64_t Nb = SEAM ? lds_ld<uint64_t>(a + 2 * RS + (P0 ? -8 : 8)) : 0ull;
+    __builtin_amdgcn_sched_barrier(0);
+    int rga = rg, rgb = rg + 1;
+    if (EDGE) edge_rows<NO>(c, to_wrap, rg, rga, rgb);
+    const u32x4 w0 = philox_vk(cq, (uint32_t)rga, hs, c.tag_hi, K);
+    const u32x4 w1 = philox_vk(cq, (uint32_t)rgb, hs, c.tag_hi, K);
+    __builtin_amdgcn_sched_barrier(0);
+    const uint32_t C0l = (uint32_t)R1, C0h = (uint32_t)(R1 >> 32), C1l = (uint32_t)R2, C1h = (uint32_t)(R2 >> 32);
+    uint32_t S0l = P0 ? __builtin_amdgcn_alignbyte(C0h, C0l, 1) : __builtin_amdgcn_alignbyte(C0l, A0, 3);
+    uint32_t S0h = P0 ? __builtin_amdgcn_alignbyte(A0, C0h, 1) : __builtin_amdgcn_alignbyte(C0h, C0l, 3);
+    uint32_t S1l = P0 ? __builtin_amdgcn_alignbyte(C1l, A1, 3) : __builtin_amdgcn_alignbyte(C1h, C1l, 1);
+    uint32_t S1h = P0 ? __builtin_amdgcn_alignbyte(C1h, C1l, 3) : __builtin_amdgcn_alignbyte(A1, C1h, 1);
+    if (SEAM) {
+        const uint64_t nxa = (Na & 0xFFull) << c.sh_next, pva = (Na >> c.sh_prev) & 0xFFull;
+        const uint64_t nxb = (Nb & 0xFFull) << c.sh_next, pvb = (Nb >> c.sh_prev) & 0xFFull;
+        const uint64_t Sa = P0 ? ((R1 >> 8) | nxa) : ((R1 << 8) | pva);
+        const uint64_t Sb = P0 ? ((R2 << 8) | pvb) : ((R2 >> 8) | nxb);
+        S0l = (uint32_t)Sa; S0h = (uint32_t)(Sa >> 32);
+        S1l = (uint32_t)Sb; S1h = (uint32_t)(Sb >> 32);
+    }
+    const uint32_t ml = C0l + C1l, mh = C0h + C1h;
+    const uint32_t cnt0l = (uint32_t)R0 + ml + S0l, cnt0h = (uint32_t)(R0 >> 32) + mh + S0h;
+    const uint32_t cnt1l = (uint32_t)R3 + ml + S1l, cnt1h = (uint32_t)(R3 >> 32) + mh + S1h;
+    u32x4 d0, d1;
+    uint32_t edge_a = 0, edge_b = 0;
+    if (OPEN) {
+        const bool ea = rga == 0 || rga == c.last_row, eb = rgb == 0 || rgb == c.last_row;
+        const bool la = !P0 && c.lft, ra = c.rgt && c.r_par == (uint32_t)P0, lb = P0 && c.lft, rb = c.rgt && c.r_par != (uint32_t)P0;
+        d0 = compare_octet_open(w0, cnt0l, cnt0h, c, ea, la, ra);
+        d1 = compare_octet_open(w1, cnt1l, cnt1h, c, eb, lb, rb);
+        edge_a = (ea ? 1u : 0u) | (la ? 2u : 0u) | (ra ? 4u : 0u) | (c.r_slot << 4);
+        edge_b = (eb ? 1u : 0u) | (lb ? 2u : 0u) | (rb ? 4u : 0u) | (c.r_slot << 4);
+    } else {
+        d0 = compare_octet(w0, cnt0l, cnt0h, c.tblH0, c.tblH1, c.tblL0, c.tblL1);
+        d1 = compare_octet(w1, cnt1l, cnt1h, c.tblH0, c.tblH1, c.tblL0, c.tblL1);
+    }
+    const uint32_t mn = minu16(minu16(minu16(d0.x, d0.y), minu16(d0.z, d0.w)), minu16(minu16(d1.x, d1.y), minu16(d1.z, d1.w)));
+    if (__builtin_expect(((mn & 0xFFFFu) == 0) | ((mn >> 16) == 0), 0)) {
+        if (has_zero_field(d0)) d0 = resolve_ties(d0, w0, cnt0l, cnt0h, c.s_thr, cq, (uint32_t)rga, hs, c.tag_lo, c.k0, c.k1, edge_a);
+        if (has_zero_field(d1)) d1 = resolve_ties(d1, w1, cnt1l, cnt1h, c.s_thr, cq, (uint32_t)rgb, hs, c.tag_lo, c.k0, c.k1, edge_b);
+    }
+    uint64_t n0 = pack_flags(d0), n1 = pack_flags(d1);
+    if (OPEN) {
+        n0 = (rga < 0 || rga > c.last_row) ? 0 : (n0 & (P0 ? c.vm_o : c.vm_e));
+        n1 = (rgb < 0 || rgb > c.last_row) ? 0 : (n1 & (P0 ? c.vm_e : c.vm_o));
+    }
+    if (SEAM) {
+        n0 &= c.vm_e;
+        n1 &= c.vm_e;
+    }
+    lds_st<uint64_t>(a + RS + DO, n0);
+    lds_st<uint64_t>(a + 2 * RS + DO, n1);
+}
+
+template <int NO, int RL, int KAPPA, int P0, bool EDGE, bool OPEN, bool SEAM = false>
+static __device__ __forceinline__ void sweep_pairs(const Rows2Ctx& c, const PhiloxKeys& K, uint32_t hs, uint32_t a, int rg, int n, bool tail,
                                                    uint32_t cq) {
-    const char* const ps0 = reinterpret_cast<const char*>(c.Ps);
-    const int d_off = (int)(reinterpret_cast<const char*>(c.Pd) - ps0);
-    const int off_end = tr_end * NO * 8;
-    const int off_step = step_rows * NO * 8;
-    int off = (tr_first * NO + oct) * 8;
-    int rg = EDGE ? tr_first : c.rgf + (tr_first - c.tr_lo);
     int to_wrap = EDGE ? c.wrap_tr - __builtin_amdgcn_readfirstlane(rg) : 0;
+    bool live = true;
 #pragma unroll 1
-    for (; off < off_end; off += off_step, rg += step_rows, to_wrap -= step_rows) {
-        asm volatile("" : "+v"(off), "+v"(rg));
-        const char* ps = ps0 + off;
-        const uint64_t R0 = *reinterpret_cast<const uint64_t*>(ps - NO * 8), R1 = *reinterpret_cast<const uint64_t*>(ps);
-        const uint64_t R2 = *reinterpret_cast<const uint64_t*>(ps + NO * 8), R3 = *reinterpret_cast<const uint64_t*>(ps + 2 * NO * 8);
-        const uint32_t A0 = SEAM ? 0u : *reinterpret_cast<const uint32_t*>(ps + (P0 ? 8 : -4));
-        const uint32_t A1 = SEAM ? 0u : *reinterpret_cast<const uint32_t*>(ps + NO * 8 + (P0 ? -4 : 8));
-        const uint64_t Na = SEAM ? *reinterpret_cast<const uint64_t*>(ps + (P0 ? 8 : -8)) : 0ull;
-        const uint64_t Nb = SEAM ? *reinterpret_cast<const uint64_t*>(ps + NO * 8 + (P0 ? -8 : 8)) : 0ull;
-        __builtin_amdgcn_sched_barrier(0);
-        int rga = rg, rgb = rg + 1;
-        if (EDGE) edge_rows<NO>(c, to_wrap, rg, rga, rgb);
-        const u32x4 w0 = philox_vk(cq, (uint32_t)rga, c.hs, c.tag_hi, K);
-        const u32x4 w1 = philox_vk(cq, (uint32_t)rgb, c.hs, c.tag_hi, K);
-        __builtin_amdgcn_sched_barrier(0);
-        const uint32_t C0l = (uint32_t)R1, C0h = (uint32_t)(R1 >> 32), C1l = (uint32_t)R2, C1h = (uint32_t)(R2 >> 32);
-        uint32_t S0l = P0 ? __builtin_amdgcn_alignbyte(C0h, C0l, 1) : __builtin_amdgcn_alignbyte(C0l, A0, 3);
-        uint32_t S0h = P0 ? __builtin_amdgcn_alignbyte(A0, C0h, 1) : __builtin_amdgcn_alignbyte(C0h, C0l, 3);
-        uint32_t S1l = P0 ? __builtin_amdgcn_alignbyte(C1l, A1, 3) : __builtin_amdgcn_alignbyte(C1h, C1l, 1);
-        uint32_t S1h = P0 ? __builtin_amdgcn_alignbyte(C1h, C1l, 3) : __builtin_amdgcn_alignbyte(A1, C1h, 1);
-        if (SEAM) {
-            const uint64_t nxa = (Na & 0xFFull) << c.sh_next, pva = (Na >> c.sh_prev) & 0xFFull;
-            const uint64_t nxb = (Nb & 0xFFull) << c.sh_next, pvb = (Nb >> c.sh_prev) & 0xFFull;
-            const uint64_t Sa = P0 ? ((R1 >> 8) | nxa) : ((R1 << 8) | pva);
-            const uint64_t Sb = P0 ? ((R2 << 8) | pvb) : ((R2 >> 8) | nxb);
-            S0l = (uint32_t)Sa; S0h = (uint32_t)(Sa >> 32);
-            S1l = (uint32_t)Sb; S1h = (uint32_t)(Sb >> 32);
-        }
-        const uint32_t ml = C0l + C1l, mh = C0h + C1h;
-        const uint32_t cnt0l = (uint32_t)R0 + ml + S0l, cnt0h = (uint32_t)(R0 >> 32) + mh + S0h;
-        const uint32_t cnt1l = (uint32_t)R3 + ml + S1l, cnt1h = (uint32_t)(R3 >> 32) + mh + S1h;
-        u32x4 d0, d1;
-        uint32_t edge_a = 0, edge_b = 0;
-        if (OPEN) {
-            const bool ea = rga == 0 || rga == c.last_row, eb = rgb == 0 || rgb == c.last_row;
-            const bool la = !P0 && c.lft, ra = c.rgt && c.r_par == (uint32_t)P0, lb = P0 && c.lft, rb = c.rgt && c.r_par != (uint32_t)P0;
-            d0 = compare_octet_open(w0, cnt0l, cnt0h, c, ea, la, ra);
-            d1 = compare_octet_open(w1, cnt1l, cnt1h, c, eb, lb, rb);
-            edge_a = (ea ? 1u : 0u) | (la ? 2u : 0u) | (ra ? 4u : 0u) | (c.r_slot << 4);
-            edge_b = (eb ? 1u : 0u) | (lb ? 2u : 0u) | (rb ? 4u : 0u) | (c.r_slot << 4);
-        } else {
-            d0 = compare_octet(w0, cnt0l, cnt0h, c.tblH0, c.tblH1, c.tblL0, c.tblL1);
-            d1 = compare_octet(w1, cnt1l, cnt1h, c.tblH0, c.tblH1, c.tblL0, c.tblL1);
-        }
-        const uint32_t mn = minu16(minu16(minu16(d0.x, d0.y), minu16(d0.z, d0.w)), minu16(minu16(d1.x, d1.y), minu16(d1.z, d1.w)));
-        if (__builtin_expect(((mn & 0xFFFFu) == 0) | ((mn >> 16) == 0), 0)) {
-            if (has_zero_field(d0)) d0 = resolve_ties(d0, w0, cnt0l, cnt0h, c.s_thr, cq, (uint32_t)rga, c.hs, c.tag_lo, c.k0, c.k1, edge_a);
-            if (has_zero_field(d1)) d1 = resolve_ties(d1, w1, cnt1l, cnt1h, c.s_thr, cq, (uint32_t)rgb, c.hs, c.tag_lo, c.k0, c.k1, edge_b);
-        }
-        char* pd = const_cast<char*>(ps) + d_off;
-        uint64_t n0 = pack_flags(d0), n1 = pack_flags(d1);
-        if (OPEN) {
-            n0 = (rga < 0 || rga > c.last_row) ? 0 : (n0 & (P0 ? c.vm_o : c.vm_e));
-            n1 = (rgb < 0 || rgb > c.last_row) ? 0 : (n1 & (P0 ? c.vm_e : c.vm_o));
-        }
-        if (SEAM) {
-            n0 &= c.vm_e;
-            n1 &= c.vm_e;
-        }
-        *reinterpret_cast<uint64_t*>(pd) = n0;
-        *reinterpret_cast<uint64_t*>(pd + NO * 8) = n1;
+    for (int i = n; i >= 0; --i) {
+        if (i == 0) live = tail;
+        asm volatile("" : "+v"(a), "+v"(rg));
+        if (live) pair_step<NO, KAPPA, P0, EDGE, OPEN, SEAM>(c, K, hs, a, rg, to_wrap, cq);
+        a += 2 * RL * 2 * NO * 8;
+        rg += 2 * RL;
+        to_wrap -= 2 * RL;
     }
 }
 
@@ -269,70 +284,108 @@
     return (uint32_t)f | ((uint32_t)(f >> 32) << 4);
 }
 
-template <int NO, int P0, bool EDGE, bool OPEN = false, bool SEAM = false>
-static __device__ __forceinline__ void sweep_pairs_nib(const Rows2Ctx& c, const PhiloxKeys& K, int tr_first, int tr_end, int step_rows, int oct,
+template <int NO, int KAPPA, int P0, bool EDGE, bool OPEN, bool SEAM>
+static __device__ __forceinline__ void pair_step_nib(const Rows2Ctx& c, const PhiloxKeys& K, uint32_t hs, uint32_t a, int rg, int to_wrap,
+                                                     uint32_t cq) {
+    constexpr int RS = 2 * NO * 4;
+    constexpr int DO = (KAPPA ? NO : -NO) * 4;
+    const uint32_t R0 = lds_ld<uint32_t>(a), R1 = lds_ld<uint32_t>(a + RS);
+    const uint32_t R2 = lds_ld<uint32_t>(a + 2 * RS), R3 = lds_ld<uint32_t>(a + 3 * RS);
+    const uint32_t A0 = lds_ld<uint32_t>(a + RS + (P0 ? 4 : -4));
+    const uint32_t A1 = lds_ld<uint32_t>(a + 2 * RS + (P0 ? -4 : 4));
+    __builtin_amdgcn_sched_barrier(0);
+    int rga = rg, rgb = rg + 1;
+    if (EDGE) edge_rows<NO>(c, to_wrap, rg, rga, rgb);
+    const u32x4 w0 = philox_vk(cq, (uint32_t)rga, hs, c.tag_hi, K);
+    const u32x4 w1 = philox_vk(cq, (uint32_t)rgb, hs, c.tag_hi, K);
+    __builtin_amdgcn_sched_barrier(0);
+    const uint32_t Sa = SEAM ? (P0 ? nib_shift_next_seam(R1, A0, c.sh_next) : nib_shift_prev_seam(R1, A0, c.sh_prev))
+                             : (P0 ? nib_shift_next(R1, A0) : nib_shift_prev(R1, A0));
+    const uint32_t Sb = SEAM ? (P0 ? nib_shift_prev_seam(R2, A1, c.sh_prev) : nib_shift_next_seam(R2, A1, c.sh_next))
+                             : (P0 ? nib_shift_prev(R2, A1) : nib_shift_next(R2, A1));
+    const uint32_t mid = R1 + R2;
+    const uint32_t cnt0 = R0 + mid + Sa, cnt1 = R3 + mid + Sb;
+    const uint32_t cnt0l = cnt0 & 0x0F0F0F0Fu, cnt0h = (cnt0 >> 4) & 0x0F0F0F0Fu;
+    const uint32_t cnt1l = cnt1 & 0x0F0F0F0Fu, cnt1h = (cnt1 >> 4) & 0x0F0F0F0Fu;
+    u32x4 d0, d1;
+    uint32_t edge_a = 0, edge_b = 0;
+    if (OPEN) {
+        const bool ea = rga == 0 || rga == c.last_row, eb = rgb == 0 || rgb == c.last_row;
+        const bool la = !P0 && c.lft, ra = c.rgt && c.r_par == (uint32_t)P0, lb = P0 && c.lft, rb = c.rgt && c.r_par != (uint32_t)P0;
+        d0 = compare_octet_open(w0, cnt0l, cnt0h, c, ea, la, ra);
+        d1 = compare_octet_open(w1, cnt1l, cnt1h, c, eb, lb, rb);
+        edge_a = (ea ? 1u : 0u) | (la ? 2u : 0u) | (ra ? 4u : 0u) | (c.r_slot << 4);
+        edge_b = (eb ? 1u : 0u) | (lb ? 2u : 0u) | (rb ? 4u : 0u) | (c.r_slot << 4);
+    } else {
+        d0 = compare_octet(w0, cnt0l, cnt0h, c.tblH0, c.tblH1, c.tblL0, c.tblL1);
+        d1 = compare_octet(w1, cnt1l, cnt1h, c.tblH0, c.tblH1, c.tblL0, c.tblL1);
+    }
+    const uint32_t mn = minu16(minu16(minu16(d0.x, d0.y), minu16(d0.z, d0.w)), minu16(minu16(d1.x, d1.y), minu16(d1.z, d1.w)));
+    if (__builtin_expect(((mn & 0xFFFFu) == 0) | ((mn >> 16) == 0), 0)) {
+        if (has_zero_field(d0)) d0 = resolve_ties(d0, w0, cnt0l, cnt0h, c.s_thr, cq, (uint32_t)rga, hs, c.tag_lo, c.k0, c.k1, edge_a);
+        if (has_zero_field(d1)) d1 = resolve_ties(d1, w1, cnt1l, cnt1h, c.s_thr, cq, (uint32_t)rgb, hs, c.tag_lo, c.k0, c.k1, edge_b);
+    }
+    uint32_t n0 = nib_pack(d0), n1 = nib_pack(d1);
+    if (OPEN) {
+        n0 = (rga < 0 || rga > c.last_row) ? 0u : (n0 & (P0 ? c.nvm_o : c.nvm_e));
+        n1 = (rgb < 0 || rgb > c.last_row) ? 0u : (n1 & (P0 ? c.nvm_e : c.nvm_o));
+    }
+    if (SEAM) {
+        n0 &= c.nvm_e;
+        n1 &= c.nvm_e;
+    }
+    lds_st<uint32_t>(a + RS + DO, n0);
+    lds_st<uint32_t>(a + 2 * RS + DO, n1);
+}
+
+template <int NO, int RL, int KAPPA, int P0, bool EDGE, bool OPEN = false, bool SEAM = false>
+static __device__ __forceinline__ void sweep_pairs_nib(const Rows2Ctx& c, const PhiloxKeys& K, uint32_t hs, uint32_t a, int rg, int n, bool tail,
                                                        uint32_t cq) {
-    const char* const ps0 = reinterpret_cast<const char*>(c.Ps);
-    const int d_off = (int)(reinterpret_cast<const char*>(c.Pd) - ps0);
-    const int off_end = tr_end * NO * 4;
-    const int off_step = step_rows * NO * 4;
-    int off = (tr_first * NO + oct) * 4;
-    int rg = EDGE ? tr_first : c.rgf + (tr_first - c.tr_lo);
     int to_wrap = EDGE ? c.wrap_tr - __builtin_amdgcn_readfirstlane(rg) : 0;
+    bool live = true;
 #pragma unroll 1
-    for (; off < off_end; off += off_step, rg += step_rows, to_wrap -= step_rows) {
-        asm volatile("" : "+v"(off), "+v"(rg));
-        const char* ps = ps0 + off;
-        const uint32_t R0 = *reinterpret_cast<const uint32_t*>(ps - NO * 4), R1 = *reinterpret_cast<const uint32_t*>(ps);
-        const uint32_t R2 = *reinterpret_cast<const uint32_t*>(ps + NO * 4), R3 = *reinterpret_cast<const uint32_t*>(ps + 2 * NO * 4);
-        const uint32_t A0 = *reinterpret_cast<const uint32_t*>(ps + (P0 ? 4 : -4));
-        const uint32_t A1 = *reinterpret_cast<const uint32_t*>(ps + NO * 4 + (P0 ? -4 : 4));
-        __builtin_amdgcn_sched_barrier(0);
-        int rga = rg, rgb = rg + 1;
-        if (EDGE) edge_rows<NO>(c, to_wrap, rg, rga, rgb);
-        const u32x4 w0 = philox_vk(cq, (uint32_t)rga, c.hs, c.tag_hi, K);
-        const u32x4 w1 = philox_vk(cq, (uint32_t)rgb, c.hs, c.tag_hi, K);
-        __builtin_amdgcn_sched_barrier(0);
-        const uint32_t Sa = SEAM ? (P0 ? nib_shift_next_seam(R1, A0, c.sh_next) : nib_shift_prev_seam(R1, A0, c.sh_prev))
-                                 : (P0 ? nib_shift_next(R1, A0) : nib_shift_prev(R1, A0));
-        const uint32_t Sb = SEAM ? (P0 ? nib_shift_prev_seam(R2, A1, c.sh_prev) : nib_shift_next_seam(R2, A1, c.sh_next))
-                                 : (P0 ? nib_shift_prev(R2, A1) : nib_shift_next(R2, A1));
-        const uint32_t mid = R1 + R2;
-        const uint32_t cnt0 = R0 + mid + Sa, cnt1 = R3 + mid + Sb;
-        const uint32_t cnt0l = cnt0 & 0x0F0F0F0Fu, cnt0h = (cnt0 >> 4) & 0x0F0F0F0Fu;
-        const uint32_t cnt1l = cnt1 & 0x0F0F0F0Fu, cnt1h = (cnt1 >> 4) & 0x0F0F0F0Fu;
-        u32x4 d0, d1;
-        uint32_t edge_a = 0, edge_b = 0;
-        if (OPEN) {
-            const bool ea = rga == 0 || rga == c.last_row, eb = rgb == 0 || rgb == c.last_row;
-            const bool la = !P0 && c.lft, ra = c.rgt && c.r_par == (uint32_t)P0, lb = P0 && c.lft, rb = c.rgt && c.r_par != (uint32_t)P0;
-            d0 = compare_octet_open(w0, cnt0l, cnt0h, c, ea, la, ra);
-            d1 = compare_octet_open(w1, cnt1l, cnt1h, c, eb, lb, rb);
-            edge_a = (ea ? 1u : 0u) | (la ? 2u : 0u) | (ra ? 4u : 0u) | (c.r_slot << 4);
-            edge_b = (eb ? 1u : 0u) | (lb ? 2u : 0u) | (rb ? 4u : 0u) | (c.r_slot << 4);
+    for (int i = n; i >= 0; --i) {
+        if (i == 0) live = tail;
+        asm volatile("" : "+v"(a), "+v"(rg));
+        if (live) pair_step_nib<NO, KAPPA, P0, EDGE, OPEN, SEAM>(c, K, hs, a, rg, to_wrap, cq);
+        a += 2 * RL * 2 * NO * 4;
+        rg += 2 * RL;
+        to_wrap -= 2 * RL;
+    }
+}
+
+template <int NO, int RL, int KAPPA, int P0, bool EDGE, bool OPEN, bool SEAM, bool NIB>
+static __device__ __forceinline__ void half_sweep(const Rows2Ctx& c, const PhiloxKeys& K, int TR, uint32_t sweep, int s, uint32_t a_thr, int al,
+                                                  uint32_t cq) {
+    constexpr int ES = NIB ? 4 : 8;
+    const int hsi = 2 * s + KAPPA;
+    __syncthreads();
+    if (al < RL) {
+        const int npairs = (TR - 2 - 2 * hsi) / 2;
+        const int n = __builtin_amdgcn_readfirstlane(npairs / RL);
+        const bool tail = al < npairs - n * RL;
+        const uint32_t a = a_thr + (uint32_t)(hsi * 2 * NO * ES + (KAPPA ? 0 : NO * ES));
+        int rg;
+        if (EDGE) {
+            rg = 1 + hsi + 2 * al;
         } else {
-            d0 = compare_octet(w0, cnt0l, cnt0h, c.tblH0, c.tblH1, c.tblL0, c.tblL1);
-            d1 = compare_octet(w1, cnt1l, cnt1h, c.tblH0, c.tblH1, c.tblL0, c.tblL1);
-        }
-        const uint32_t mn = minu16(minu16(minu16(d0.x, d0.y), minu16(d0.z, d0.w)), minu16(minu16(d1.x, d1.y), minu16(d1.z, d1.w)));
-        if (__builtin_expect(((mn & 0xFFFFu) == 0) | ((mn >> 16) == 0), 0)) {
-            if (has_zero_field(d0)) d0 = resolve_ties(d0, w0, cnt0l, cnt0h, c.s_thr, cq, (uint32_t)rga, c.hs, c.tag_lo, c.k0, c.k1, edge_a);
-            if (has_zero_field(d1)) d1 = resolve_ties(d1, w1, cnt1l, cnt1h, c.s_thr, cq, (uint32_t)rgb, c.hs, c.tag_lo, c.k0, c.k1, edge_b);
-        }
-        char* pd = const_cast<char*>(ps) + d_off;
-        uint32_t n0 = nib_pack(d0), n1 = nib_pack(d1);
-        if (OPEN) {
-            const uint64_t ma = P0 ? c.vm_o : c.vm_e, mb = P0 ? c.vm_e : c.vm_o;
-            n0 = (rga < 0 || rga > c.last_row) ? 0u : (n0 & ((uint32_t)ma | ((uint32_t)(ma >> 32) << 4)));
-            n1 = (rgb < 0 || rgb > c.last_row) ? 0u : (n1 & ((uint32_t)mb | ((uint32_t)(mb >> 32) << 4)));
-        }
-        if (SEAM) {
-            const uint32_t m = (uint32_t)c.vm_e | ((uint32_t)(c.vm_e >> 32) << 4);
-            n0 &= m;
-            n1 &= m;
-        }
-        *reinterpret_cast<uint32_t*>(pd) = n0;
-        *reinterpret_cast<uint32_t*>(pd + NO * 4) = n1;
+            int rgf = c.rg_tile0 + 1 + hsi;
+            if (!OPEN && rgf >= c.total_rows) rgf -= c.total_rows;
+            rg = rgf + 2 * al;
+        }
+        const uint32_t hs = 2u * sweep + (uint32_t)KAPPA;
+        if constexpr (NIB) sweep_pairs_nib<NO, RL, KAPPA, P0, EDGE, OPEN, SEAM>(c, K, hs, a, rg, n, tail, cq);
+        else sweep_pairs<NO, RL, KAPPA, P0, EDGE, OPEN, SEAM>(c, K, hs, a, rg, n, tail, cq);
+    }
+}
+
+template <int NO, int RL, int P0, bool EDGE, bool OPEN, bool SEAM, bool NIB>
+static __device__ __forceinline__ void sweep_generation(const Rows2Ctx& c, const PhiloxKeys& K, int TR, uint32_t sweep_g, int kg, uint32_t a_thr,
+                                                        int al, uint32_t cq) {
+#pragma unroll 1
+    for (int s = 0; s < kg; ++s) {
+        half_sweep<NO, RL, 0, P0, EDGE, OPEN, SEAM, NIB>(c, K, TR, sweep_g + (uint32_t)s, s, a_thr, al, cq);
+        half_sweep<NO, RL, 1, P0, EDGE, OPEN, SEAM, NIB>(c, K, TR, sweep_g + (uint32_t)s, s, a_thr, al, cq);
     }
 }
 
@@ -364,9 +417,8 @@
     const int TR = H + 4 * k;
     constexpr int RL = RLMAX;
     using E = typename std::conditional<NIB, uint32_t, uint64_t>::type;
-    E* plane0 = reinterpret_cast<E*>(lds + 1);
-    E* plane1 = plane0 + TR * NO;
-    uint64_t* s_thr = reinterpret_cast<uint64_t*>((reinterpret_cast<uintptr_t>(plane1 + TR * NO + NO + 1) + 7u) & ~(uintptr_t)7u);
+    const TilePlanes<E, NO> P{reinterpret_cast<E*>(lds + 1)};
+    uint64_t* s_thr = reinterpret_cast<uint64_t*>((reinterpret_cast<uintptr_t>(P.base + 2 * TR * NO + NO + 1) + 7u) & ~(uintptr_t)7u);
     const int tid = threadIdx.x;
     if (tid < 25) s_thr[tid] = p.thr[tid];
 
@@ -417,14 +469,13 @@
                         ev &= vm_e;
                         od &= vm_o;
                     }
-                    const int idx = tr * NO + oct;
                     const int gpar = (int)((p.row0 + Rb + tr) & 1);
                     if (NIB) {
-                        (gpar ? plane1 : plane0)[idx] = (E)((uint32_t)ev | ((uint32_t)(ev >> 32) << 4));
-                        (gpar ? plane0 : plane1)[idx] = (E)((uint32_t)od | ((uint32_t)(od >> 32) << 4));
+                        P.at(gpar, tr, oct) = (E)((uint32_t)ev | ((uint32_t)(ev >> 32) << 4));
+                        P.at(gpar ^ 1, tr, oct) = (E)((uint32_t)od | ((uint32_t)(od >> 32) << 4));
                     } else {
-                        (gpar ? plane1 : plane0)[idx] = (E)ev;
-                        (gpar ? plane0 : plane1)[idx] = (E)od;
+                        P.at(gpar, tr, oct) = (E)ev;
+                        P.at(gpar ^ 1, tr, oct) = (E)od;
                     }
                 }
             }
@@ -453,8 +504,10 @@
     c.r_slot = ((uint32_t)(p.cols - 1) & 15u) >> 1;
     c.rm_lo = c.r_slot < 4 ? 0xFFu << (8 * c.r_slot) : 0u;
     c.rm_hi = c.r_slot < 4 ? 0u : 0xFFu << (8 * (c.r_slot - 4));
-    c.vm_e = vm_e;
-    c.vm_o = vm_o;
+    c.vm_e = NIB ? 0 : vm_e;
+    c.vm_o = NIB ? 0 : vm_o;
+    c.nvm_e = NIB ? ((uint32_t)vm_e | ((uint32_t)(vm_e >> 32) << 4)) : 0u;
+    c.nvm_o = NIB ? ((uint32_t)vm_o | ((uint32_t)(vm_o >> 32) << 4)) : 0u;
     const int v_last = (p.cols >> 1) & 7;
     const bool ragged = !OPEN && v_last != 0;
     const int seam_site = v_last - 1;
@@ -497,12 +550,12 @@
         const uint64_t tag = strip_tag(gen);
         for (int i = tid; i < n_tb; i += THREADS) {
             const int r = i / WO, o = i - r * WO;
-            xst(mine + i, (uint64_t)plane1[(2 * k + r) * NO + 1 + o] | tag);
-            xst(mine + n_tb + i, (uint64_t)plane1[(H + r) * NO + 1 + o] | tag);
+            xst(mine + i, (uint64_t)P.at(1, 2 * k + r, 1 + o) | tag);
+            xst(mine + n_tb + i, (uint64_t)P.at(1, H + r, 1 + o) | tag);
         }
         for (int i = tid; i < n_lr; i += THREADS) {
-            xst(mine + 2 * n_tb + i, (uint64_t)plane1[(2 * k + i) * NO + 1] | tag);
-            xst(mine + 2 * n_tb + n_lr + i, (uint64_t)plane1[(2 * k + i) * NO + wi] | tag);
+            xst(mine + 2 * n_tb + i, (uint64_t)P.at(1, 2 * k + i, 1) | tag);
+            xst(mine + 2 * n_tb + n_lr + i, (uint64_t)P.at(1, 2 * k + i, wi) | tag);
         }
         RES_MARK(1);
     };
@@ -579,71 +632,45 @@
             const int i = tid + it * THREADS;
             if (i < 2 * k * NO) {
                 const int r = i / NO, o = i - r * NO;
-                if (nu[it]) plane1[r * NO + o] = (E)(vu[it] & FLAG_MASK);
-                if (nd[it]) plane1[(2 * k + H + r) * NO + o] = (E)(vd[it] & FLAG_MASK);
+                if (nu[it]) P.at(1, r, o) = (E)(vu[it] & FLAG_MASK);
+                if (nd[it]) P.at(1, 2 * k + H + r, o) = (E)(vd[it] & FLAG_MASK);
             }
         }
 #pragma unroll
         for (int it = 0; it < SI; ++it) {
             const int i = tid + it * THREADS;
             if (i < n_lr) {
-                if (nl[it]) plane1[(2 * k + i) * NO] = (E)(vl[it] & FLAG_MASK);
-                if (nr[it]) plane1[(2 * k + i) * NO + wi + 1] = (E)(vr[it] & FLAG_MASK);
+                if (nl[it]) P.at(1, 2 * k + i, 0) = (E)(vl[it] & FLAG_MASK);
+                if (nr[it]) P.at(1, 2 * k + i, wi + 1) = (E)(vr[it] & FLAG_MASK);
             }
         }
         RES_MARK(3);
     };
 
-    auto run = [&](int par0, int tr_first, int tr_end, int step, int oc, uint32_t cqq) {
-        if (NIB && OPEN) {
-            if (par0) sweep_pairs_nib<NO, 1, false, true>(c, K, tr_first, tr_end, step, oc, cqq);
-            else sweep_pairs_nib<NO, 0, false, true>(c, K, tr_first, tr_end, step, oc, cqq);
-        } else if (NIB && seam) {
-            if (par0) sweep_pairs_nib<NO, 1, true, false, true>(c, K, tr_first, tr_end, step, oc, cqq);
-            else sweep_pairs_nib<NO, 0, true, false, true>(c, K, tr_first, tr_end, step, oc, cqq);
-        } else if (NIB) {
-            if (edge) {
-                if (par0) sweep_pairs_nib<NO, 1, true>(c, K, tr_first, tr_end, step, oc, cqq);
-                else sweep_pairs_nib<NO, 0, true>(c, K, tr_first, tr_end, step, oc, cqq);
-            } else {
-                if (par0) sweep_pairs_nib<NO, 1, false>(c, K, tr_first, tr_end, step, oc, cqq);
-                else sweep_pairs_nib<NO, 0, false>(c, K, tr_first, tr_end, step, oc, cqq);
+    const int par0 = (int)((p.row0 + Rb + 1) & 1);
+    const int form = 2 * (OPEN ? 0 : (seam ? 1 : (edge ? 2 : 3))) + par0;
+    const uint32_t a_thr = lds_addr(P.base) + (uint32_t)((4 * al * NO + oct) * (int)sizeof(E));
+    auto run_generation = [&](uint32_t sweep_g, int kg) {
+#define TSU_FORM(P0, EDGE_, OPEN_, SEAM_) sweep_generation<NO, RL, P0, EDGE_, OPEN_, SEAM_, NIB>(c, K, TR, sweep_g, kg, a_thr, al, cq)
+        if constexpr (OPEN) {
+            if (par0) TSU_FORM(1, false, true, false);
+            else TSU_FORM(0, false, true, false);
+        } else {
+            switch (form) {
+                case 2: TSU_FORM(0, true, false, true); break;
+                case 3: TSU_FORM(1, true, false, true); break;
+                case 4: TSU_FORM(0, true, false, false); break;
+                case 5: TSU_FORM(1, true, false, false); break;
+                case 6: TSU_FORM(0, false, false, false); break;
+                default: TSU_FORM(1, false, false, false); break;
             }
-        } else if (OPEN) {
-            if (par0) sweep_pairs<NO, 1, false, true>(c, K, tr_first, tr_end, step, oc, cqq);
-            else sweep_pairs<NO, 0, false, true>(c, K, tr_first, tr_end, step, oc, cqq);
-        } else if (seam) {
-            if (par0) sweep_pairs<NO, 1, true, false, true>(c, K, tr_first, tr_end, step, oc, cqq);
-            else sweep_pairs<NO, 0, true, false, true>(c, K, tr_first, tr_end, step, oc, cqq);
-        } else if (edge) {
-            if (par0) sweep_pairs<NO, 1, true, false>(c, K, tr_first, tr_end, step, oc, cqq);
-            else sweep_pairs<NO, 0, true, false>(c, K, tr_first, tr_end, step, oc, cqq);
-        } else {
-            if (par0) sweep_pairs<NO, 1, false, false>(c, K, tr_first, tr_end, step, oc, cqq);
-            else sweep_pairs<NO, 0, false, false>(c, K, tr_first, tr_end, step, oc, cqq);
-        }
-    };
-    int par0 = 0;
-    auto set_half_sweep = [&](uint32_t sweep_g, int hsi) {
-        const int kappa = hsi & 1;
-        c.hs = 2u * (sweep_g + (uint32_t)(hsi >> 1)) + (uint32_t)kappa;
-        c.Pd = kappa ? plane1 : plane0;
-        c.Ps = kappa ? plane0 : plane1;
-        c.tr_lo = 1 + hsi;
-        c.npairs = (TR - 2 - 2 * hsi) / 2;
-        int rgf = (int)rg0 + c.tr_lo;
-        if (!OPEN && rgf >= c.total_rows) rgf -= c.total_rows;
-        c.rgf = rgf;
-        par0 = (int)((p.row0 + Rb + c.tr_lo + kappa) & 1);
+        }
+#undef TSU_FORM
     };
     for (int gen = 0; gen < n_gen; ++gen) {
     const int kg = (RESIDENT && gen == n_gen - 1) ? R->k_last : k;
     const uint32_t sweep_g = sweep0 + (uint32_t)(gen * k);
-    for (int hsi = 0; hsi < 2 * kg; ++hsi) {
-        __syncthreads();
-        set_half_sweep(sweep_g, hsi);
-        if (al < RL) run(par0, c.tr_lo + 2 * al, c.tr_lo + 2 * c.npairs, 2 * RL, oct, cq);
-    }
+    run_generation(sweep_g, kg);
     __syncthreads();
     if (RESIDENT && gen + 1 < n_gen) {
         publish(gen);
@@ -663,8 +690,7 @@
         for (int hr = al; hr < H; hr += RLMAX) {
             const int rl = r0 + hr;
             if (rl < p.r_end) {
-                const int li = (2 * k + hr) * NO + oct;
-                uint64_t ev = (gpar ? plane1 : plane0)[li], od = (gpar ? plane0 : plane1)[li];
+                uint64_t ev = P.at(gpar, 2 * k + hr, oct), od = P.at(gpar ^ 1, 2 * k + hr, oct);
                 if (NIB) {
                     ev = (ev & 0x01010101ull) | (((ev >> 4) & 0x01010101ull) << 32);
                     od = (od & 0x01010101ull) | (((od >> 4) & 0x01010101ull) << 32);
```

Measured after the change: 3168 billion (median of 6 runs). +5.0%, better.
